# Dylan102938/distributed-llm-inference

Measured on AMD Instinct MI355X. Metric: output tokens/sec (whole node) + p50 token latency, Llama-3-70B PP=8, higher is better.
Workload: dtype bf16; 1 GPU; model=Llama-3-70B, global_batch=512, seq_len=647, parallelism=pp1

## Files before the change

distributed_llm_inference/config.py:

```python
from __future__ import annotations

import dataclasses
import json
import math
import os
from dataclasses import dataclass, field
from typing import Any, Dict, List, Optional, Sequence, Tuple


@dataclass(frozen=True)
class ModelSpec:

    arch: str = "llama"
    vocab_size: int = 128256
    hidden_size: int = 4096
    intermediate_size: int = 14336
    num_layers: int = 32
    num_heads: int = 32
    num_kv_heads: int = 8
    head_dim: int = 128
    rms_norm_eps: float = 1e-5
    rope_theta: float = 500000.0
    rope_scaling: Optional[Tuple[Tuple[str, Any], ...]] = None
    max_position_embeddings: int = 8192
# ... 247 lines not shown
        raise ValueError("num_stages must be >= 1")
    if num_stages > L:
        raise ValueError(f"cannot split {L} layers into {num_stages} stages")
    w = list(weights) if weights is not None else [1.0] * num_stages
    if len(w) != num_stages or min(w) <= 0:
        raise ValueError("weights must be positive, one per stage")
    head_cost = 0.6 * spec.vocab_size * spec.hidden_size / max(1, spec.layer_param_count())
    extra = [0.0] * num_stages
    if num_stages > 1:
        if head_rotation:
            extra = [head_cost / num_stages] * num_stages
        else:
            extra[-1] += head_cost
    total = (L + sum(extra))
    tw = sum(w)
    targets = [total * wi / tw - ei for wi, ei in zip(w, extra)]
    counts = [max(1, int(math.floor(t))) for t in targets]
    while sum(counts) > L:
        i = max((k for k in range(num_stages) if counts[k] > 1),
                key=lambda k: (counts[k] + extra[k]) / w[k])
        counts[i] -= 1
    while sum(counts) < L:
        i = min(range(num_stages), key=lambda k: ((counts[k] + 1 + extra[k]) / w[k], k))
        counts[i] += 1
    out, s = [], 0
    for c in counts:
        out.append((s, s + c))
        s += c
    return out


@dataclass
class CacheConfig:

    block_size: int = 64
    num_blocks: Optional[int] = None
    gpu_memory_utilization: float = 0.90
    window_length: int = 0
    num_sink_tokens: int = 0
    max_chunk: int = 512
    dtype: str = "bf16"
    k_scale: float = 1.0
    v_scale: float = 1.0

    def __post_init__(self):
        if self.dtype not in ("bf16", "fp8"):
            raise ValueError(f"KV cache dtype must be 'bf16' or 'fp8', got {self.dtype!r}")

    @property
    def windowed(self) -> bool:
        return self.window_length > 0

    @property
    def torch_dtype(self):
        import torch
        return torch.float8_e4m3fn if self.dtype == "fp8" else torch.bfloat16

    @property
    def dtype_bytes(self) -> int:
        return 1 if self.dtype == "fp8" else 2


@dataclass
class KernelPolicy:

    gemm4: bool = True
    fp8_gemm4: str = "gate_up"
    gemm4_decode_sched: int = 8
    bf16_partials: bool = True
    defer_splitk: bool = True
    fp8_mx: bool = True
    tile_gemms: bool = True
    library_gemms: Optional[bool] = None
    tile_gemm_max_m: int = 2048
    warm_library_gemms: bool = True
    stream_k_tail: bool = False
    gemv: bool = True
    gemv_norm: bool = True
    int8_transposed: bool = False
    prefill_m32: bool = True
    fp4_mfma: bool = False
    fp4_small_m: int = 0
    fp8_small_m: int = 0

    _FP8_SHAPES = ("qkv", "o", "gate_up", "down")

    def __post_init__(self):
        if self.fp4_small_m != 0 and not 3 <= self.fp4_small_m <= 32:
            raise ValueError(f"fp4_small_m={self.fp4_small_m}: 0 (off) or 3..32")
        if self.fp8_small_m != 0 and not 3 <= self.fp8_small_m <= 32:
            raise ValueError(f"fp8_small_m={self.fp8_small_m}: 0 (off) or 3..32")
        if self.gemm4_decode_sched not in (4, 6, 8, 9):
            raise ValueError(f"gemm4_decode_sched={self.gemm4_decode_sched}: 4, 6, 8 or 9")
        sel = self.fp8_gemm4
        if sel not in ("all", "none") and any(
                x not in self._FP8_SHAPES for x in sel.split("+")):
            raise ValueError(f"fp8_gemm4={sel!r}: 'all', 'none' or a '+' list of "
                             f"{'/'.join(self._FP8_SHAPES)}")

    def fp8_on_gemm4(self, shape: str) -> bool:
        return self.gemm4 and (self.fp8_gemm4 == "all" or shape in self.fp8_gemm4.split("+"))

    def with_overrides(self, spec: str) -> "KernelPolicy":
        if not spec or not spec.strip():
            return self
        kw: Dict[str, Any] = {}
        names = {f.name: f for f in dataclasses.fields(self)}
        for item in spec.split(","):
            if not item.strip():
                continue
            k, _, v = item.partition("=")
            k, v = k.strip(), v.strip()
            if k not in names:
                raise ValueError(f"unknown kernel policy field {k!r} (known: {sorted(names)})")
            if k == "fp8_gemm4":
                kw[k] = v
            elif names[k].type in (int, "int"):
                kw[k] = int(v)
            elif k == "library_gemms" and v.lower() in ("auto", "none", ""):
                kw[k] = None
            elif v.lower() in ("1", "true", "on", "yes"):
                kw[k] = True
            elif v.lower() in ("0", "false", "off", "no"):
                kw[k] = False
            else:
                raise ValueError(f"kernel policy {k}={v!r}: expected 0/1")
        return dataclasses.replace(self, **kw)


@dataclass
class ServeConfig:
    max_batch_size: int = 256
    max_num_batched_tokens: int = 8192
    num_micro_batches: int = 0
    max_seq_len: int = 8192
    use_graphs: bool = True
    head_rotation: bool = True
    graph_batch_sizes: List[int] = field(default_factory=lambda: [1, 2, 4, 8, 16, 32, 64, 96, 128,
                                                                  160, 192, 224, 256])
```

distributed_llm_inference/csrc/bindings.hip:

```cpp
#include <torch/extension.h>
#include <ATen/hip/HIPContext.h>
#include <ATen/hip/impl/HIPGuardImplMasqueradingAsCUDA.h>
#include <ATen/hip/impl/HIPStreamMasqueradingAsCUDA.h>

#include <cstdlib>

#include "kernels/kernels.h"

using at::Tensor;
using c10::optional;

namespace {

#define CHECK_DEV(t) TORCH_CHECK((t).is_cuda(), #t " must be a GPU tensor")
#define CHECK_CONTIG(t) TORCH_CHECK((t).is_contiguous(), #t " must be contiguous")
#define CHECK_BF16(t) TORCH_CHECK((t).scalar_type() == at::kBFloat16, #t " must be bfloat16")
#define CHECK_I32(t) TORCH_CHECK((t).scalar_type() == at::kInt, #t " must be int32")
#define CHECK_I64(t) TORCH_CHECK((t).scalar_type() == at::kLong, #t " must be int64")
#define CHECK_F32(t) TORCH_CHECK((t).scalar_type() == at::kFloat, #t " must be float32")
#define CHECK_IN(t) \
  CHECK_DEV(t);     \
  CHECK_CONTIG(t)

inline dli::bf16* bp(const Tensor& t) { return reinterpret_cast<dli::bf16*>(t.data_ptr()); }
// ... 22 lines not shown
      ro = bp(*residual_out);
    }
  }
  const c10::hip::HIPGuardMasqueradingAsCUDA g(x.device());
  check_rc(dli::launch_rms_norm(bp(out), bp(x), r, ro, bp(w), (float)eps, (int)rows, (int)hidden,
                                cur_stream()), "rms_norm");
}

void splitk_reduce(Tensor out, Tensor parts) {
  CHECK_IN(out); CHECK_IN(parts); CHECK_BF16(out); CHECK_F32(parts);
  TORCH_CHECK(parts.dim() == 3 && out.numel() == parts.size(1) * parts.size(2),
              "splitk_reduce: parts [S, M, N] and out [M, N]");
  const c10::hip::HIPGuardMasqueradingAsCUDA g(parts.device());
  check_rc(dli::launch_splitk_reduce(bp(out), parts.data_ptr<float>(), (int)parts.size(0),
                                     (size_t)out.numel(), cur_stream()), "splitk_reduce");
}

void rms_norm_splitk(Tensor out, Tensor parts, optional<Tensor> residual, Tensor w, double eps,
                     optional<Tensor> residual_out) {
  CHECK_IN(out); CHECK_IN(parts); CHECK_IN(w);
  CHECK_BF16(out); CHECK_BF16(w);
  const bool parts_bf16 = parts.scalar_type() == at::kBFloat16;
  TORCH_CHECK(parts_bf16 || parts.scalar_type() == at::kFloat, "rms_norm_splitk: fp32 or bf16 parts");
  TORCH_CHECK(parts.dim() == 3, "rms_norm_splitk: parts must be [splits, rows, hidden]");
  const int64_t splits = parts.size(0), rows = parts.size(1), hidden = parts.size(2);
  TORCH_CHECK(splits >= 1 && w.numel() == hidden && out.numel() == rows * hidden,
              "rms_norm_splitk: shape mismatch");
  const dli::bf16* r = nullptr;
  dli::bf16* ro = nullptr;
  if (residual.has_value()) {
    CHECK_IN(*residual); CHECK_BF16(*residual);
    TORCH_CHECK(residual->numel() == rows * hidden, "rms_norm_splitk: residual shape mismatch");
    r = bp(*residual);
    ro = bp(*residual);
    if (residual_out.has_value()) {
      CHECK_IN(*residual_out); CHECK_BF16(*residual_out);
      TORCH_CHECK(residual_out->numel() == rows * hidden, "rms_norm_splitk: residual_out shape");
      ro = bp(*residual_out);
    }
  }
  const c10::hip::HIPGuardMasqueradingAsCUDA g(parts.device());
  check_rc(dli::launch_rms_norm(bp(out), nullptr, r, ro, bp(w), (float)eps, (int)rows,
                                (int)hidden, cur_stream(), parts.data_ptr(), (int)splits,
                                parts_bf16),
           "rms_norm_splitk");
}

void layer_norm(Tensor out, Tensor x, optional<Tensor> residual, Tensor w, Tensor b, double eps,
                optional<Tensor> residual_out) {
  CHECK_IN(out); CHECK_IN(x); CHECK_IN(w); CHECK_IN(b);
  CHECK_BF16(out); CHECK_BF16(x); CHECK_BF16(w); CHECK_BF16(b);
  const int64_t hidden = x.size(-1);
  const int64_t rows = x.numel() / hidden;
  TORCH_CHECK(w.numel() == hidden && b.numel() == hidden && out.numel() == x.numel(),
              "layer_norm: shape mismatch");
  const dli::bf16* r = nullptr;
  dli::bf16* ro = nullptr;
  if (residual.has_value()) {
    CHECK_IN(*residual); CHECK_BF16(*residual);
    TORCH_CHECK(residual->numel() == x.numel(), "layer_norm: residual shape mismatch");
    r = bp(*residual);
    ro = bp(*residual);
    if (residual_out.has_value()) {
      CHECK_IN(*residual_out); CHECK_BF16(*residual_out);
      TORCH_CHECK(residual_out->numel() == x.numel(), "layer_norm: residual_out shape mismatch");
      ro = bp(*residual_out);
    }
  }
  const c10::hip::HIPGuardMasqueradingAsCUDA g(x.device());
  check_rc(dli::launch_layer_norm(bp(out), bp(x), r, ro, bp(w), bp(b), (float)eps, (int)rows,
                                  (int)hidden, cur_stream()), "layer_norm");
}

void silu_mul(Tensor out, Tensor x, bool interleaved) {
  CHECK_IN(out); CHECK_IN(x); CHECK_BF16(out); CHECK_BF16(x);
  const int64_t two_i = x.size(-1);
  TORCH_CHECK(two_i % 2 == 0, "silu_mul: last dim must be even");
  const int64_t rows = x.numel() / two_i;
  TORCH_CHECK(out.numel() == rows * (two_i / 2), "silu_mul: out shape mismatch");
  const c10::hip::HIPGuardMasqueradingAsCUDA g(x.device());
  check_rc(dli::launch_silu_mul(bp(out), bp(x), (int)rows, (int)(two_i / 2), interleaved,
                                cur_stream()),
           "silu_mul");
}

void gelu_bias(Tensor out, Tensor x, optional<Tensor> bias) {
  CHECK_IN(out); CHECK_IN(x); CHECK_BF16(out); CHECK_BF16(x);
  const int64_t cols = x.size(-1);
  const int64_t rows = x.numel() / cols;
  TORCH_CHECK(out.numel() == x.numel(), "gelu: out shape mismatch");
  dli::bf16* bb = nullptr;
  if (bias.has_value()) {
    CHECK_IN(*bias); CHECK_BF16(*bias);
    TORCH_CHECK(bias->numel() == cols, "gelu: bias shape mismatch");
    bb = bp(*bias);
  }
  const c10::hip::HIPGuardMasqueradingAsCUDA g(x.device());
  check_rc(dli::launch_gelu_bias(bp(out), bp(x), bb, (int)rows, (int)cols, cur_stream()), "gelu");
}

void add(Tensor out, Tensor a, Tensor b) {
  CHECK_IN(out); CHECK_IN(a); CHECK_IN(b);
  CHECK_BF16(out); CHECK_BF16(a); CHECK_BF16(b);
  TORCH_CHECK(a.numel() == b.numel() && out.numel() == a.numel(), "add: shape mismatch");
  const c10::hip::HIPGuardMasqueradingAsCUDA g(a.device());
  check_rc(dli::launch_add(bp(out), bp(a), bp(b), (size_t)a.numel(), cur_stream()), "add");
}

bool check_cache(const Tensor& k_cache, const Tensor& v_cache, int64_t nkv, int64_t D) {
  CHECK_IN(k_cache); CHECK_IN(v_cache);
  const bool fp8 = k_cache.scalar_type() == at::kFloat8_e4m3fn;
  TORCH_CHECK(fp8 || k_cache.scalar_type() == at::kBFloat16, "KV cache must be bf16 or fp8 e4m3fn");
  TORCH_CHECK(v_cache.scalar_type() == k_cache.scalar_type(), "k/v caches must share a dtype");
  TORCH_CHECK(k_cache.dim() == 4 && v_cache.dim() == 5, "k_cache must be 4-D, v_cache 5-D");
  TORCH_CHECK(k_cache.size(1) == nkv && k_cache.size(3) == D, "k_cache must be [blocks, nkv, bs, D]");
  TORCH_CHECK(v_cache.size(0) == k_cache.size(0) && v_cache.size(1) == nkv &&
                  v_cache.size(2) * 8 == k_cache.size(2) && v_cache.size(3) == D &&
                  v_cache.size(4) == 8,
              "v_cache must be [blocks, nkv, bs/8, D, 8]");
  return fp8;
}

void rope_cache(Tensor qkv, optional<Tensor> positions, optional<Tensor> slot_mapping,
                optional<Tensor> cos_sin, Tensor q_out, optional<Tensor> q_sink_out,
                int64_t window, Tensor k_cache, Tensor v_cache, int64_t nh, int64_t nkv,
                double k_scale, double v_scale) {
  CHECK_DEV(qkv);
  const bool parts_bf16 = qkv.scalar_type() == at::kBFloat16 && qkv.dim() == 3;
  const bool parts = qkv.scalar_type() == at::kFloat || parts_bf16;
  if (parts) {
    TORCH_CHECK(qkv.dim() == 3 && qkv.is_contiguous(), "qkv partials must be contiguous [S, T, N]");
  } else {
    CHECK_BF16(qkv);
    TORCH_CHECK(qkv.dim() == 2 && qkv.stride(1) == 1, "qkv must be [T, *] with unit inner stride");
  }
  const int64_t T = parts ? qkv.size(1) : qkv.size(0);
  CHECK_IN(q_out); CHECK_BF16(q_out);
  TORCH_CHECK(q_out.dim() == 3 && q_out.size(0) == T && q_out.size(1) == nh, "q_out must be [T, nh, D]");
  const int64_t D = q_out.size(2);
  TORCH_CHECK(qkv.size(qkv.dim() - 1) >= (nh + 2 * nkv) * D, "qkv too narrow for nh/nkv/D");
  const bool fp8 = check_cache(k_cache, v_cache, nkv, D);
  TORCH_CHECK(k_scale > 0 && v_scale > 0, "KV scales must be positive");
  dli::RopeCacheParams p{};
  p.kv_fp8 = fp8 ? 1 : 0;
  p.k_inv_scale = (float)(1.0 / k_scale);
  p.v_inv_scale = (float)(1.0 / v_scale);
  if (parts) {
    p.qkv = nullptr;
    p.qkv_parts = qkv.data_ptr();
    p.parts_bf16 = parts_bf16 ? 1 : 0;
    p.splits = (int)qkv.size(0);
    p.qkv_stride = qkv.size(2);
    p.split_stride = (long)(T * qkv.size(2));
  } else {
    p.qkv = bp(qkv);
    p.qkv_stride = qkv.stride(0);
  }
  if (positions.has_value()) {
    CHECK_IN(*positions); CHECK_I32(*positions);
    TORCH_CHECK(positions->numel() == T, "positions must have T entries");
    p.positions = positions->data_ptr<int>();
  }
  if (slot_mapping.has_value()) {
    CHECK_IN(*slot_mapping); CHECK_I64(*slot_mapping);
    TORCH_CHECK(slot_mapping->numel() == T, "slot_mapping must have T entries");
    p.slot_mapping = reinterpret_cast<const long*>(slot_mapping->data_ptr<int64_t>());
// ... 29 lines not shown
                            double k_scale, double v_scale, int64_t& D,
                            bool allow_empty_out = false) {
  CHECK_IN(out); CHECK_IN(q); CHECK_BF16(out); CHECK_BF16(q);
  TORCH_CHECK(q.dim() == 3, "q must be [T, nh, D]");
  TORCH_CHECK(out.sizes() == q.sizes() || (allow_empty_out && out.numel() == 0),
              "out must match q");
  const int64_t nh = q.size(1);
  D = q.size(2);
  const int64_t nkv = k_cache.size(1);
  TORCH_CHECK(nkv > 0 && nh % nkv == 0, "nh must be a multiple of nkv");
  const bool fp8 = check_cache(k_cache, v_cache, nkv, D);
  TORCH_CHECK(k_scale > 0 && v_scale > 0, "KV scales must be positive");
  CHECK_IN(block_tables); CHECK_I32(block_tables); CHECK_IN(seq_lens); CHECK_I32(seq_lens);
  TORCH_CHECK(block_tables.dim() == 2 && block_tables.size(0) == seq_lens.size(0),
              "block_tables must be [B, max_blocks]");
  dli::AttnParams p{};
  p.q = bp(q);
  if (ring > 0) {
    TORCH_CHECK(q_sink.has_value() || n_sink == 0, "window mode with sinks needs q_sink");
    TORCH_CHECK(window > n_sink && sink_pad >= n_sink && sink_pad % 32 == 0 && ring % 32 == 0,
                "invalid window configuration");
  }
  if (q_sink.has_value()) {
    CHECK_IN(*q_sink); CHECK_BF16(*q_sink);
    TORCH_CHECK(q_sink->sizes() == q.sizes(), "q_sink must match q");
    p.q_sink = bp(*q_sink);
  }
  p.k_cache = k_cache.data_ptr();
  p.v_cache = v_cache.data_ptr();
  p.kv_fp8 = fp8 ? 1 : 0;
  p.k_scale = (float)k_scale;
  p.v_scale = (float)v_scale;
  p.out = out.numel() ? bp(out) : nullptr;
  p.block_tables = block_tables.data_ptr<int>();
  p.bt_stride = (int)block_tables.size(1);
  p.seq_lens = seq_lens.data_ptr<int>();
  p.scale_log2 = (float)(scale * 1.4426950408889634);
  p.nh = (int)nh;
  p.nkv = (int)nkv;
  p.bs = (int)k_cache.size(2);
  p.n_sink = (int)n_sink;
  p.sink_pad = (int)sink_pad;
  p.ring = (int)ring;
  p.window = (int)window;
  p.num_splits = 1;
  TORCH_CHECK(p.bs % 32 == 0, "cache block size must be a multiple of 32");
  return p;
}

void attn_decode(Tensor out, Tensor q, optional<Tensor> q_sink, Tensor k_cache, Tensor v_cache,
                 Tensor block_tables, Tensor seq_lens, double scale, int64_t n_sink,
                 int64_t sink_pad, int64_t ring, int64_t window, int64_t num_splits,
                 optional<Tensor> part_o, optional<Tensor> part_ml, double k_scale,
                 double v_scale, optional<Tensor> out_q, optional<Tensor> out_mx) {
  int64_t D = 0;
  auto p = attn_common(out, q, q_sink, k_cache, v_cache, block_tables, seq_lens, scale, n_sink,
                       sink_pad, ring, window, k_scale, v_scale, D, out_q.has_value());
  const int64_t B = q.size(0);
  TORCH_CHECK(seq_lens.numel() == B, "decode: one token per sequence (seq_lens must have T entries)");
  TORCH_CHECK(num_splits >= 1, "num_splits >= 1");
  p.num_splits = (int)num_splits;
  TORCH_CHECK(out_q.has_value() == out_mx.has_value(), "attn_decode: out_q and out_mx go together");
  if (out_q.has_value()) {
    CHECK_IN(*out_q); CHECK_IN(*out_mx);
    TORCH_CHECK(D == 128 && num_splits == 1, "attn_decode: MX output needs head_dim 128, one split");
    TORCH_CHECK(out_q->element_size() == 1 && out_q->numel() == B * p.nh * D,
                "attn_decode: out_q = fp8 [T, nh * D]");
    TORCH_CHECK(out_mx->element_size() == 1 && out_mx->numel() == p.nh * ((B + 63) / 64) * 64,
                "attn_decode: out_mx = e8m0 [nh][ceil(T / 64) * 64]");
    p.out_q = static_cast<uint8_t*>(out_q->data_ptr());
    p.out_mx = static_cast<uint8_t*>(out_mx->data_ptr());
  }
  if (num_splits > 1) {
    TORCH_CHECK(part_o.has_value() && part_ml.has_value(), "split-K needs workspaces");
    CHECK_IN(*part_o); CHECK_IN(*part_ml); CHECK_F32(*part_o); CHECK_F32(*part_ml);
    TORCH_CHECK(part_o->numel() >= num_splits * B * p.nh * D, "part_o workspace too small");
    TORCH_CHECK(part_ml->numel() >= num_splits * B * p.nh * 2, "part_ml workspace too small");
    p.part_o = part_o->data_ptr<float>();
    p.part_ml = part_ml->data_ptr<float>();
  }
  const c10::hip::HIPGuardMasqueradingAsCUDA g(q.device());
  check_rc(dli::launch_attn_decode(p, (int)B, (int)D, cur_stream()), "attn_decode");
}

void attn_prefill(Tensor out, Tensor q, optional<Tensor> q_sink, Tensor k_cache, Tensor v_cache,
                  Tensor block_tables, Tensor seq_lens, Tensor q_start, int64_t max_q,
                  double scale, int64_t n_sink, int64_t sink_pad, int64_t ring, int64_t window,
                  double k_scale, double v_scale, optional<Tensor> tile_map, int64_t qb,
                  optional<Tensor> mask, bool m32) {
  int64_t D = 0;
  auto p = attn_common(out, q, q_sink, k_cache, v_cache, block_tables, seq_lens, scale, n_sink,
                       sink_pad, ring, window, k_scale, v_scale, D);
  CHECK_IN(q_start); CHECK_I32(q_start);
  const int64_t B = seq_lens.numel();
  TORCH_CHECK(q_start.numel() == B + 1, "q_start must have B+1 entries");
  p.q_start = q_start.data_ptr<int>();
  if (tile_map.has_value()) {
    CHECK_IN(*tile_map); CHECK_I32(*tile_map);
    TORCH_CHECK(tile_map->dim() == 2 && tile_map->size(1) == 2, "tile_map must be [n_tiles, 2]");
    p.tile_map = tile_map->data_ptr<int>();
    p.n_tiles = (int)tile_map->size(0);
  }
  TORCH_CHECK(qb == 1 || qb == 2, "attn_prefill: qb (query blocks per wave) must be 1 or 2");
  p.prefill_qb = (int)qb;
  p.prefill_m32 = m32 ? 1 : 0;
  if (mask.has_value()) {
    CHECK_IN(*mask); CHECK_F32(*mask);
    TORCH_CHECK(mask->dim() == 4 && mask->size(0) == B &&
                    (mask->size(1) == 1 || mask->size(1) == q.size(1)),
                "attn_prefill: mask must be [B, 1 | nh, T, keys]");
    TORCH_CHECK(ring == 0 && !tile_map.has_value(),
                "attn_prefill: a custom mask needs a full cache and the dense grid");
    p.mask = mask->data_ptr<float>();
    p.mask_heads = (int)mask->size(1);
    p.mask_q = (int)mask->size(2);
    p.mask_k = (int)mask->size(3);
  }
  const c10::hip::HIPGuardMasqueradingAsCUDA g(q.device());
  check_rc(dli::launch_attn_prefill(p, (int)B, (int)max_q, (int)D, cur_stream()), "attn_prefill");
}

void sample(Tensor out_tokens, optional<Tensor> out_logprobs, Tensor logits,
            optional<Tensor> temperature, optional<Tensor> top_k, optional<Tensor> top_p,
            optional<Tensor> seeds, optional<Tensor> step, optional<Tensor> ctr) {
  CHECK_DEV(logits);
  TORCH_CHECK(logits.dim() == 2 && logits.stride(1) == 1, "logits must be [B, V] row-major");
  TORCH_CHECK(logits.scalar_type() == at::kBFloat16 || logits.scalar_type() == at::kFloat,
              "logits must be bf16 or f32");
  const int64_t B = logits.size(0);
  CHECK_IN(out_tokens); CHECK_I32(out_tokens);
  TORCH_CHECK(out_tokens.numel() == B, "out_tokens must have B entries");
  dli::SampleParams p{};
  p.logits = logits.data_ptr();
  p.logits_is_f32 = logits.scalar_type() == at::kFloat;
  p.row_stride = logits.stride(0);
  p.V = (int)logits.size(1);
  auto opt_f = [&](optional<Tensor>& t, const char* n) -> const float* {
    if (!t.has_value()) return nullptr;
    CHECK_IN(*t); CHECK_F32(*t);
    TORCH_CHECK(t->numel() == B, n, " must have B entries");
    return t->data_ptr<float>();
  };
  p.temperature = opt_f(temperature, "temperature");
  p.top_p = opt_f(top_p, "top_p");
  if (top_k.has_value()) {
    CHECK_IN(*top_k); CHECK_I32(*top_k);
    TORCH_CHECK(top_k->numel() == B, "top_k must have B entries");
    p.top_k = top_k->data_ptr<int>();
  }
  if (seeds.has_value()) {
    CHECK_IN(*seeds); CHECK_I64(*seeds);
    TORCH_CHECK(seeds->numel() == B, "seeds must have B entries");
    p.seeds = reinterpret_cast<const unsigned long long*>(seeds->data_ptr<int64_t>());
  }
  if (step.has_value()) {
    CHECK_IN(*step); CHECK_I64(*step);
    p.step = reinterpret_cast<const long*>(step->data_ptr<int64_t>());
  }
  if (ctr.has_value()) {
    CHECK_IN(*ctr); CHECK_I64(*ctr);
    TORCH_CHECK(ctr->numel() == B, "ctr must have B entries");
    p.ctr = reinterpret_cast<const long*>(ctr->data_ptr<int64_t>());
  }
  p.out_tokens = out_tokens.data_ptr<int>();
  if (out_logprobs.has_value()) {
    CHECK_IN(*out_logprobs); CHECK_F32(*out_logprobs);
// ... 606 lines not shown
  }
  TORCH_CHECK(M >= 1 && M <= 2 && (fp4 || w.size(1) == K) && q_out.size(0) == M &&
                  q_out.size(1) == nh && N == (nh + 2 * nkv) * D,
              "skinny_gemm_qkv_rope: x [M <= 2, K], w [(nh + 2 nkv) D, K], q_out [M, nh, D]");
  const bool fp8 = check_cache(k_cache, v_cache, nkv, D);
  TORCH_CHECK(k_scale > 0 && v_scale > 0, "KV scales must be positive");
  dli::GemvRope rp{};
  rp.kv_fp8 = fp8 ? 1 : 0;
  rp.k_inv_scale = (float)(1.0 / k_scale);
  rp.v_inv_scale = (float)(1.0 / v_scale);
  if (positions.has_value()) {
    CHECK_IN(*positions); CHECK_I32(*positions);
    TORCH_CHECK(positions->numel() == M, "positions must have M entries");
    rp.positions = positions->data_ptr<int>();
  }
  if (slot_mapping.has_value()) {
    CHECK_IN(*slot_mapping); CHECK_I64(*slot_mapping);
    TORCH_CHECK(slot_mapping->numel() == M, "slot_mapping must have M entries");
    rp.slot_mapping = reinterpret_cast<const long*>(slot_mapping->data_ptr<int64_t>());
  }
  if (cos_sin.has_value()) {
    CHECK_IN(*cos_sin); CHECK_F32(*cos_sin);
    TORCH_CHECK(cos_sin->dim() == 2 && cos_sin->size(1) == D && positions.has_value(),
                "cos_sin must be [max_pos, D] (with positions)");
    rp.cos_sin = cos_sin->data_ptr<float>();
    rp.max_pos = (int)cos_sin->size(0);
  }
  rp.q_out = bp(q_out);
  rp.k_cache = k_cache.data_ptr();
  rp.v_cache = v_cache.data_ptr();
  rp.nh = (int)nh;
  rp.nkv = (int)nkv;
  rp.D = (int)D;
  rp.bs = (int)k_cache.size(2);
  const GemvNormArgs na = gemv_norm_args(x, norm_w, res_in, res_out, eps, "skinny_gemm_qkv_rope");
  const dli::GemvNorm* nm = na.on ? &na.nm : nullptr;
  const dli::bf16* b = nullptr;
  if (bias.has_value()) {
    CHECK_IN(*bias); CHECK_BF16(*bias);
    TORCH_CHECK(bias->numel() == N, "skinny_gemm_qkv_rope: bias must have N entries");
    b = bp(*bias);
  }
  const c10::hip::HIPGuardMasqueradingAsCUDA g(x.device());
  int rc;
  if (fp4) {
    rc = dli::launch_skinny_gemm_fp4(nullptr, bp(x), w.data_ptr<uint8_t>(),
                                     block_scale->data_ptr<uint8_t>(), b, (int)M, (int)N, (int)K,
                                     cur_stream(), false, nm, &rp);
  } else if (w.scalar_type() == at::kBFloat16) {
    rc = dli::launch_skinny_gemm(nullptr, bp(x), bp(w), b, (int)M, (int)N, (int)K, cur_stream(),
                                 false, nm, &rp);
  } else {
    TORCH_CHECK(wscale.has_value() && w.element_size() == 1, "8-bit weights need wscale");
    CHECK_IN(*wscale); CHECK_F32(*wscale);
    TORCH_CHECK(wscale->numel() == N, "wscale must have N entries");
    if (w.scalar_type() == at::kChar)
      rc = dli::launch_skinny_gemm_int8(nullptr, bp(x), w.data_ptr<int8_t>(),
                                        wscale->data_ptr<float>(), b, (int)M, (int)N, (int)K,
                                        cur_stream(), false, nm, &rp);
    else
      rc = dli::launch_skinny_gemm_fp8(nullptr, x.data_ptr(), nullptr,
                                       static_cast<const uint8_t*>(w.data_ptr()),
                                       wscale->data_ptr<float>(), b, (int)M, (int)N, (int)K,
                                       cur_stream(), false, nm, &rp);
  }
  check_rc(rc, "skinny_gemm_qkv_rope");
}


}

void register_rccl(pybind11::module_& m);
void register_streams(pybind11::module_& m);

PYBIND11_MODULE(TORCH_EXTENSION_NAME, m) {
  m.doc() = "CDNA4 (gfx950) kernels of distributed_llm_inference";
  m.def("rms_norm", &rms_norm, "RMSNorm (+fused residual add)", py::arg("out"), py::arg("x"),
        py::arg("residual"), py::arg("w"), py::arg("eps"), py::arg("residual_out") = py::none());
  m.def("layer_norm", &layer_norm, "LayerNorm (+fused residual add)", py::arg("out"),
        py::arg("x"), py::arg("residual"), py::arg("w"), py::arg("b"), py::arg("eps"),
        py::arg("residual_out") = py::none());
  m.def("silu_mul", &silu_mul, "SwiGLU: out = silu(x[:, :I]) * x[:, I:] (or tile-interleaved)",
        py::arg("out"), py::arg("x"), py::arg("interleaved") = false);
  m.def("gelu_bias", &gelu_bias, "gelu_tanh(x + bias)");
  m.def("add", &add, "out = a + b");
  m.def("rope_cache", &rope_cache, "fused RoPE + paged KV cache write");
  m.def("attn_decode", &attn_decode, "paged GQA decode attention (split-K)", py::arg("out"),
        py::arg("q"), py::arg("q_sink"), py::arg("k_cache"), py::arg("v_cache"),
        py::arg("block_tables"), py::arg("seq_lens"), py::arg("scale"), py::arg("n_sink"),
        py::arg("sink_pad"), py::arg("ring"), py::arg("window"), py::arg("num_splits"),
        py::arg("part_o"), py::arg("part_ml"), py::arg("k_scale"), py::arg("v_scale"),
        py::arg("out_q") = py::none(), py::arg("out_mx") = py::none());
  m.def("attn_prefill", &attn_prefill, "paged causal prefill attention (varlen)", py::arg("out"),
        py::arg("q"), py::arg("q_sink"), py::arg("k_cache"), py::arg("v_cache"),
        py::arg("block_tables"), py::arg("seq_lens"), py::arg("q_start"), py::arg("max_q"),
        py::arg("scale"), py::arg("n_sink"), py::arg("sink_pad"), py::arg("ring"),
        py::arg("window"), py::arg("k_scale"), py::arg("v_scale"), py::arg("tile_map"),
        py::arg("qb"), py::arg("mask") = py::none(), py::arg("m32") = true);
  m.def("sample", &sample, "greedy / temperature / top-k / top-p sampling", py::arg("out_tokens"),
        py::arg("out_logprobs"), py::arg("logits"), py::arg("temperature"), py::arg("top_k"),
        py::arg("top_p"), py::arg("seeds"), py::arg("step"), py::arg("ctr") = py::none());
  m.def("digest", &digest, "hop-integrity payload digest partials", py::arg("part"), py::arg("t"));
  m.def("quant_rowwise", &quant_rowwise, "row-wise fp8 e4m3 quantisation (+fused RMSNorm)",
        py::arg("q_out"), py::arg("scale"), py::arg("x"), py::arg("residual"), py::arg("norm_w"),
        py::arg("eps"), py::arg("residual_out") = py::none());
  m.def("quant_rowwise_int8", &quant_rowwise_int8, "LLM.int8 row-wise int8 quantisation (outlier columns zeroed)",
        py::arg("q_out"), py::arg("scale"), py::arg("x"), py::arg("outlier") = py::none());
  m.def("llm_int8_outliers", &llm_int8_outliers,
        "LLM.int8 outlier columns: (flags, x_out, w_out, cnt) for the bf16 outlier product",
        py::arg("x"), py::arg("wq"), py::arg("ws"), py::arg("threshold"), py::arg("max_out"),
        py::arg("wq_t") = py::none(), py::arg("dynamic") = false);
  m.def("silu_mul_quant", &silu_mul_quant, "SwiGLU fused with row-wise fp8 quantisation");
  m.def("gemm_tile", &gemm_tile, "C = A . B^T, 256x256 LDS-DMA 8-phase MFMA tile GEMM",
        py::arg("out"), py::arg("a"), py::arg("b"), py::arg("splits") = 1,
        py::arg("epilogue") = 0, py::arg("workspace") = py::none(),
        py::arg("a_scale") = py::none(), py::arg("b_scale") = py::none(),
        py::arg("x_out") = py::none(), py::arg("w_out") = py::none(),
        py::arg("a_mx") = py::none(), py::arg("out_mx") = py::none(),
        py::arg("ol_cnt") = py::none());
  m.def("rms_norm_splitk", &rms_norm_splitk, "residual add + RMSNorm over un-reduced split-K partials",
        py::arg("out"), py::arg("parts"), py::arg("residual"), py::arg("w"), py::arg("eps"),
        py::arg("residual_out") = py::none());
  m.def("splitk_reduce", &splitk_reduce, "bf16 out = sum of fp32 split-K partials [S, M, N]");
  m.def("gemm_tile_sk_workspace_floats", []() { return dli::gemm_tile_sk_workspace_floats(); },
        "fp32 workspace elements gemm_tile(splits=0) needs on the current device");
  m.def("skinny_gemm_qkv_rope", &skinny_gemm_qkv_rope,
        "1-2 row fused QKV GEMV with RoPE + paged KV write in its epilogue (+ fused input RMSNorm)",
        py::arg("q_out"), py::arg("x"), py::arg("w"), py::arg("wscale"), py::arg("bias"),
        py::arg("positions"), py::arg("slot_mapping"), py::arg("cos_sin"), py::arg("k_cache"),
        py::arg("v_cache"), py::arg("nh"), py::arg("nkv"), py::arg("k_scale") = 1.0,
        py::arg("v_scale") = 1.0, py::arg("norm_w") = py::none(), py::arg("res_in") = py::none(),
        py::arg("res_out") = py::none(), py::arg("eps") = 1e-5,
        py::arg("block_scale") = py::none());
  m.def("skinny_gemm_fp4", &skinny_gemm_fp4,
        "y = x . dequant(W4)^T (+ bias), MXFP4 weights, bf16 rows, M <= 2 (weight-streaming GEMV)",
        py::arg("out"), py::arg("x"), py::arg("w"), py::arg("block_scale"),
        py::arg("bias") = py::none(), py::arg("swiglu") = false, py::arg("norm_w") = py::none(),
        py::arg("res_in") = py::none(), py::arg("res_out") = py::none(), py::arg("eps") = 1e-5);
  m.def("small_gemm_fp4", &small_gemm_fp4,
        "y = x . dequant(W4)^T (+ bias), MXFP4 weights, 3-32 bf16 rows (weight-streaming MFMA GEMM)",
        py::arg("out"), py::arg("x"), py::arg("w"), py::arg("block_scale"),
        py::arg("bias") = py::none(), py::arg("swiglu") = false);
  m.def("small_gemm_fp8", &small_gemm_fp8,
        "y = (x . W8^T) * w_scale (+ bias), fp8 weights, 3-32 bf16 rows (weight-streaming MFMA GEMM)",
        py::arg("out"), py::arg("x"), py::arg("w"), py::arg("w_scale"),
        py::arg("bias") = py::none(), py::arg("swiglu") = false);
  m.def("dequant_mxfp4", &dequant_mxfp4, "bf16 [N, K] = MXFP4 nibbles [N, K / 2] * 2^(e8m0 - 127)",
        py::arg("out"), py::arg("w"), py::arg("block_scale"));
  m.def("quant_mx", &quant_mx, "MX fp8 quantiser: bf16 [M, K] -> e4m3 bytes + e8m0 per (row, 128)",
        py::arg("q"), py::arg("sc"), py::arg("x"));
  m.def("gemm_fp4", &gemm_fp4,
        "C = A . W^T, MX fp8 activations x MXFP4 weights on the mixed-format block-scaled MFMA",
        py::arg("out"), py::arg("a_q"), py::arg("a_mx"), py::arg("w"), py::arg("block_scale"),
        py::arg("splits") = 1, py::arg("epilogue") = 0, py::arg("workspace") = py::none());
  m.def("gemm_fp4_max_ktiles", []() { return dli::gemm_fp4_max_ktiles(); },
        "k-tiles (of 128) one split of gemm_fp4 may own");
  m.def("gemm4", &gemm4, "C = A . B^T, one-wave-per-SIMD 256x256 MFMA tile GEMM (gemm4.hip)",
        py::arg("out"), py::arg("a"), py::arg("b"), py::arg("splits") = 1,
        py::arg("epilogue") = 0, py::arg("grid") = 0, py::arg("a_scale") = py::none(),
        py::arg("b_scale") = py::none(), py::arg("variant") = -1, py::arg("a_mx") = py::none(),
        py::arg("out_mx") = py::none());
  m.def("skinny_gemm_int8", &skinny_gemm_int8,
        "y = (x . W8^T) * scale (+ bias), int8 weights, bf16 rows, M <= 2 (weight-streaming GEMV)",
        py::arg("out"), py::arg("x"), py::arg("w"), py::arg("wscale"), py::arg("bias") = py::none(),
        py::arg("swiglu") = false, py::arg("norm_w") = py::none(), py::arg("res_in") = py::none(),
        py::arg("res_out") = py::none(), py::arg("eps") = 1e-5);
  m.def("skinny_gemm_fp8", &skinny_gemm_fp8,
        "y = (x . W8^T) * scale (+ bias), fp8 e4m3 weights, M <= 2 (weight-streaming GEMV)",
        py::arg("out"), py::arg("x"), py::arg("xscale"), py::arg("w"), py::arg("wscale"),
        py::arg("bias") = py::none(), py::arg("swiglu") = false, py::arg("norm_w") = py::none(),
        py::arg("res_in") = py::none(), py::arg("res_out") = py::none(), py::arg("eps") = 1e-5);
  m.def("skinny_gemm", &skinny_gemm, "y = x . W^T (+ bias) for M <= 4 (weight-streaming GEMV)",
        py::arg("out"), py::arg("x"), py::arg("w"), py::arg("bias") = py::none(),
        py::arg("swiglu") = false, py::arg("norm_w") = py::none(), py::arg("res_in") = py::none(),
        py::arg("res_out") = py::none(), py::arg("eps") = 1e-5);
// ... 4 lines not shown
```

distributed_llm_inference/csrc/kernels/activation.hip:

```cpp
#include "kernels.h"

namespace dli {

template <bool INTERLEAVED>
__global__ void __launch_bounds__(256) silu_mul_kernel(bf16* __restrict__ out,
                                                       const bf16* __restrict__ x, int rows,
                                                       int inter) {
  const int nvec = inter >> 3;
  const size_t total = (size_t)rows * nvec;
  for (size_t i = blockIdx.x * (size_t)blockDim.x + threadIdx.x; i < total;
       i += (size_t)gridDim.x * blockDim.x) {
    const size_t r = i / nvec, c = i % nvec;
    const bf16* row = x + r * 2 * inter;
    bf16x8 g, u;
    if (INTERLEAVED) {
      const int o = (int)c * 8;
      const int gc = (o >> 7) * 256 + ((o & 127) >> 5) * 64 + ((o & 31) >> 4) * 32 + (o & 15);
      g = *reinterpret_cast<const bf16x8*>(row + gc);
      u = *reinterpret_cast<const bf16x8*>(row + gc + 16);
    } else {
      g = reinterpret_cast<const bf16x8*>(row)[c];
      u = reinterpret_cast<const bf16x8*>(row + inter)[c];
    }
    bf16x8 o;
#pragma unroll
    for (int j = 0; j < 8; ++j) o[j] = (bf16)(silu((float)g[j]) * (float)u[j]);
    reinterpret_cast<bf16x8*>(out + r * inter)[c] = o;
  }
}

__global__ void __launch_bounds__(256) gelu_bias_kernel(bf16* __restrict__ out,
                                                        const bf16* __restrict__ x,
                                                        const bf16* __restrict__ bias, int rows,
                                                        int cols) {
  const int nvec = cols >> 3;
  const size_t total = (size_t)rows * nvec;
  for (size_t i = blockIdx.x * (size_t)blockDim.x + threadIdx.x; i < total;
       i += (size_t)gridDim.x * blockDim.x) {
    const size_t c = i % nvec;
    const bf16x8 a = reinterpret_cast<const bf16x8*>(x)[i];
    bf16x8 o;
    if (bias) {
      const bf16x8 b = reinterpret_cast<const bf16x8*>(bias)[c];
#pragma unroll
      for (int j = 0; j < 8; ++j) o[j] = (bf16)gelu_tanh((float)a[j] + (float)b[j]);
    } else {
#pragma unroll
      for (int j = 0; j < 8; ++j) o[j] = (bf16)gelu_tanh((float)a[j]);
    }
    reinterpret_cast<bf16x8*>(out)[i] = o;
  }
}

__global__ void __launch_bounds__(256) add_kernel(bf16* __restrict__ out, const bf16* __restrict__ a,
                                                  const bf16* __restrict__ b, size_t nvec) {
  for (size_t i = blockIdx.x * (size_t)blockDim.x + threadIdx.x; i < nvec;
       i += (size_t)gridDim.x * blockDim.x) {
    const bf16x8 x = reinterpret_cast<const bf16x8*>(a)[i];
    const bf16x8 y = reinterpret_cast<const bf16x8*>(b)[i];
    bf16x8 o;
#pragma unroll
    for (int j = 0; j < 8; ++j) o[j] = (bf16)((float)x[j] + (float)y[j]);
    reinterpret_cast<bf16x8*>(out)[i] = o;
  }
}

static inline int ew_grid(size_t work) {
  size_t g = (work + 255) / 256;
  if (g > 2048) g = 2048;
  if (g < 1) g = 1;
  return (int)g;
}

int launch_silu_mul(bf16* out, const bf16* x, int rows, int inter, bool interleaved,
                    hipStream_t stream) {
  if (inter % 8 != 0 || (interleaved && inter % 128 != 0)) return -1;
  if (rows == 0) return 0;
  if (interleaved)
    silu_mul_kernel<true><<<ew_grid((size_t)rows * inter / 8), 256, 0, stream>>>(out, x, rows, inter);
  else
    silu_mul_kernel<false><<<ew_grid((size_t)rows * inter / 8), 256, 0, stream>>>(out, x, rows, inter);
  return 0;
}

int launch_gelu_bias(bf16* out, const bf16* x, const bf16* bias, int rows, int cols,
                     hipStream_t stream) {
  if (cols % 8 != 0) return -1;
  if (rows == 0) return 0;
  gelu_bias_kernel<<<ew_grid((size_t)rows * cols / 8), 256, 0, stream>>>(out, x, bias, rows, cols);
  return 0;
}

int launch_add(bf16* out, const bf16* a, const bf16* b, size_t n, hipStream_t stream) {
  if (n % 8 != 0) return -1;
  if (n == 0) return 0;
  add_kernel<<<ew_grid(n / 8), 256, 0, stream>>>(out, a, b, n / 8);
  return 0;
}

}
```

distributed_llm_inference/csrc/kernels/attention.hip:

```cpp
#include "kernels.h"
#include "attn_core.h"

#include <type_traits>

namespace dli {

template <int D, bool WIN, bool FP8, bool GRP, bool ONE = false>
__global__ void __launch_bounds__(256, (ONE ? 4 : 1))
attn_decode_kernel(AttnParams p, int items, int gs) {
  constexpr int LROW = D + 4;
  __shared__ __attribute__((aligned(16))) float lds[GRP ? 4 * 16 * (LROW + 2) : 1];
  const int wave = threadIdx.x >> 6;
  const int item_raw = blockIdx.x * 4 + wave;
  const bool live = item_raw < items;
  if (!GRP && !live) return;
  const int item = __builtin_amdgcn_readfirstlane(live ? item_raw : items - 1);
  WaveState<D> st;
  const DecodeItem di = attn_decode_item<D, WIN, FP8, false, ONE>(p, item, live, st);
  const int splits = p.num_splits, split = di.split, G = di.G, hgroups = di.hgroups;
  const int g0 = di.g0, kvh = di.kvh, b = di.b;
  const int lane = threadIdx.x & 63, col = lane & 15, h4 = lane >> 4;
  const bool col_valid = di.col_valid;
  const float vsc = di.vsc;
  float lsum = st.l;
  lsum += __shfl_xor(lsum, 16, 64);
  lsum += __shfl_xor(lsum, 32, 64);
  const size_t B = (size_t)items / ((size_t)splits * hgroups * p.nkv);
  if constexpr (!GRP) {
    if (!col_valid) return;
    const int head = kvh * G + g0 + col;
    if (splits == 1) {
      const float inv = lsum > 0.f ? vsc / lsum : 0.f;
      if constexpr (D == 128) {
        if (p.out_q != nullptr) {
          f32x4 vals[D / 16];
          int dd[D / 16];
          float a = 0.f;
#pragma unroll
          for (int u = 0; u < D / 16; ++u) {
            f32x4 o;
            o_unit<D, FP8>(st, u, h4, dd[u], o);
#pragma unroll
            for (int r = 0; r < 4; ++r) {
              vals[u][r] = (float)(bf16)(o[r] * inv);
              a = fmaxf(a, fabsf(vals[u][r]));
            }
          }
          a = fmaxf(a, __shfl_xor(a, 16, 64));
          a = fmaxf(a, __shfl_xor(a, 32, 64));
          const int k = mx_exponent(a);
          const float si = mx_inv_scale(k);
          uint8_t* qrow = p.out_q + ((size_t)b * p.nh + head) * D;
#pragma unroll
          for (int u = 0; u < D / 16; ++u) {
            const f32x4 v = vals[u] * si;
            *reinterpret_cast<unsigned*>(qrow + dd[u]) = pack4_fp8(v[0], v[1], v[2], v[3]);
          }
          if (h4 == 0) {
            const int nb = ((int)B + 63) / 64;
            p.out_mx[mx_off(head, b, nb)] = (uint8_t)(k + 127);
            if (b == (int)B - 1)
              for (int r = (int)B; r < nb * 64; ++r) p.out_mx[mx_off(head, r, nb)] = 127;
          }
          return;
        }
      }
      bf16* orow = p.out + ((size_t)b * p.nh + head) * D;
#pragma unroll
      for (int u = 0; u < D / 16; ++u) {
        int d;
        f32x4 o;
        o_unit<D, FP8>(st, u, h4, d, o);
        bf16x4 v;
#pragma unroll
        for (int r = 0; r < 4; ++r) v[r] = (bf16)(o[r] * inv);
        *reinterpret_cast<bf16x4*>(orow + d) = v;
      }
    } else {
      const size_t r0 = ((size_t)split * B + b) * p.nh + head;
      float* prow = p.part_o + r0 * D;
#pragma unroll
      for (int u = 0; u < D / 16; ++u) {
        int d;
        f32x4 o;
        o_unit<D, FP8>(st, u, h4, d, o);
        *reinterpret_cast<f32x4*>(prow + d) = o * vsc;
      }
      if (h4 == 0) {
        p.part_ml[r0 * 2] = st.m;
        p.part_ml[r0 * 2 + 1] = lsum;
      }
    }
  } else {
    float* lo = lds + (wave * 16 + col) * LROW;
    float* lml = lds + 4 * 16 * LROW;
#pragma unroll
    for (int u = 0; u < D / 16; ++u) {
      int d;
      f32x4 o;
      o_unit<D, FP8>(st, u, h4, d, o);
      *reinterpret_cast<f32x4*>(lo + d) = o;
// ... 286 lines not shown
    for (int qb = 0; qb < QB; ++qb) {
      if constexpr (MASK) {
        const int k0 = u0 + 8 * h4;
        float madd[8];
        unsigned vis = 0;
#pragma unroll
        for (int j = 0; j < 8; ++j) {
          const float mv = k0 + j < mlen ? mrow[k0 + j] : -INFINITY;
          const bool ok = mv > -1e4f;
          madd[j] = ok ? mv * minv : 0.f;
          vis |= (ok ? 1u : 0u) << j;
        }
        attn_core<D>(st[qb], qf[qb], f, sl2, [&](int j) { return ((vis >> j) & 1u) != 0; },
                     [&](int j) { return madd[j]; });
        continue;
      }
      if constexpr (!WIN) {
        attn_compute_causal<D>(st[qb], qf[qb], f, sl2, pq[qb] - (u0 + 8 * h4));
        continue;
      }
      unsigned vm = 0;
#pragma unroll
      for (int j = 0; j < 8; ++j) {
        const int u = u0 + 8 * h4 + j;
        bool ok;
        if (!WIN) {
          ok = u <= pq[qb];
        } else if (sink_step) {
          ok = u < nS && u <= pq[qb];
        } else {
          ok = (u - p.sink_pad) < seg_len;
          if (ok) {
            const int a = ring_abs(u, L, p);
            ok = a >= p.n_sink && a <= pq[qb] && (pq[qb] - a) < (p.window - p.n_sink);
          }
        }
        vm |= (ok ? 1u : 0u) << j;
      }
      if constexpr (WIN) {
        if (sink_step) {
          attn_compute<D>(st[qb], qsf[qb], f, sl2, vm);
          continue;
        }
      }
      attn_compute<D>(st[qb], qf[qb], f, sl2, vm);
    }
    if constexpr (DMA) {
      asm volatile("s_waitcnt vmcnt(0)" ::: "memory");
    } else {
      if (sidx + 1 < nsteps) swrite(buf ^ 1);
    }
    __syncthreads();
  }
#pragma unroll
  for (int qb = 0; qb < QB; ++qb) {
    float lsum = st[qb].l;
    lsum += __shfl_xor(lsum, 16, 64);
    lsum += __shfl_xor(lsum, 32, 64);
    if (col_valid[qb]) {
      const float inv = lsum > 0.f ? vsc / lsum : 0.f;
      bf16* orow = p.out + ((size_t)(qs0 + tok[qb]) * p.nh + qh) * D;
#pragma unroll
      for (int e = 0; e < D / 16; ++e) {
        bf16x4 v;
#pragma unroll
        for (int r = 0; r < 4; ++r) v[r] = (bf16)(st[qb].o[e][r] * inv);
        *reinterpret_cast<bf16x4*>(orow + 16 * e + 4 * h4) = v;
      }
    }
  }
}

static int attn_cus() {
  static int cus = [] {
    int dev = 0, n = 0;
    if (hipGetDevice(&dev) != hipSuccess ||
        hipDeviceGetAttribute(&n, hipDeviceAttributeMultiprocessorCount, dev) != hipSuccess || n <= 0)
      return 256;
    return n;
  }();
  return cus;
}

template <int D, bool WIN, bool FP8>
static void decode_grid(const AttnParams& p, int items, int gs, hipStream_t stream) {
  const int grid = (items + 3) / 4;
  if (p.num_splits > 1) {
    attn_decode_kernel<D, WIN, FP8, true><<<grid, 256, 0, stream>>>(p, items, gs);
    return;
  }
  if constexpr (!WIN) {
#ifndef ATTN_DECODE_TWO_STEP
    const long s1 = 16L * attn_cus(), s2 = 8L * attn_cus();
    const long r1 = (items + s1 - 1) / s1, r2 = (items + s2 - 1) / s2;
    if (items >= s1 && (double)items / (r1 * s1) >= (double)items / (r2 * s2)) {
      attn_decode_kernel<D, WIN, FP8, false, true><<<grid, 256, 0, stream>>>(p, items, 1);
      return;
    }
#endif
  }
  attn_decode_kernel<D, WIN, FP8, false><<<grid, 256, 0, stream>>>(p, items, 1);
}

template <int D>
static int launch_decode_d(const AttnParams& p, int B, hipStream_t stream) {
  const int G = p.nh / p.nkv;
  const int hgroups = (G + 15) / 16;
  const long items = (long)B * p.nkv * hgroups * p.num_splits;
  if (items > (1L << 30)) return -3;
  const int gs = p.num_splits % 4 == 0 ? 4 : p.num_splits % 2 == 0 ? 2 : 1;
  if (p.ring > 0) {
    if (p.kv_fp8) decode_grid<D, true, true>(p, (int)items, gs, stream);
    else decode_grid<D, true, false>(p, (int)items, gs, stream);
  } else {
    if (p.kv_fp8) decode_grid<D, false, true>(p, (int)items, gs, stream);
    else decode_grid<D, false, false>(p, (int)items, gs, stream);
  }
  if (p.num_splits > gs) {
    AttnParams pc = p;
    pc.num_splits = p.num_splits / gs;
    attn_combine_kernel<D><<<B * p.nh, 256, 0, stream>>>(pc, B);
  }
  return 0;
}

int launch_attn_decode(const AttnParams& p, int B, int D, hipStream_t stream) {
  if (B == 0) return 0;
  if (p.bs % 32 != 0 || (p.ring > 0 && (p.sink_pad % 32 != 0 || p.ring % 32 != 0))) return -2;
  switch (D) {
    case 32: return launch_decode_d<32>(p, B, stream);
    case 64: return launch_decode_d<64>(p, B, stream);
    case 128: return launch_decode_d<128>(p, B, stream);
    default: return -1;
  }
}

template <int D, bool WIN, bool FP8>
static void prefill_grid(const AttnParams& p, dim3 grid, int hpw, hipStream_t stream) {
  if constexpr (!WIN) {
    if (p.mask) {
      attn_prefill_kernel<D, false, FP8, 1, true><<<grid, 256, 0, stream>>>(p, hpw);
      return;
    }
  }
  if (p.prefill_qb == 2)
    attn_prefill_kernel<D, WIN, FP8, 2><<<grid, 256, 0, stream>>>(p, hpw);
  else
    attn_prefill_kernel<D, WIN, FP8, 1><<<grid, 256, 0, stream>>>(p, hpw);
}

template <int D>
static int launch_prefill_d(const AttnParams& p, int B, int max_q, hipStream_t stream) {
  const int G = p.nh / p.nkv;
  const int hpw = (G % 4 == 0) ? 4 : (G % 2 == 0 ? 2 : 1);
  const int tpw = 4 / hpw;
  const int tt = 16 * tpw * (p.mask ? 1 : p.prefill_qb);
  dim3 grid((max_q + tt - 1) / tt, p.nkv * (G / hpw), B);
  if (p.tile_map) {
    const long total = (long)p.n_tiles * p.nkv * (G / hpw);
    grid = dim3((unsigned)((total + 7) / 8 * 8), 1, 1);
  }
  if (grid.x == 0) return 0;
  if (p.ring > 0) {
    if (p.kv_fp8) prefill_grid<D, true, true>(p, grid, hpw, stream);
    else prefill_grid<D, true, false>(p, grid, hpw, stream);
  } else {
    if (p.kv_fp8) prefill_grid<D, false, true>(p, grid, hpw, stream);
    else prefill_grid<D, false, false>(p, grid, hpw, stream);
  }
  return 0;
}

int launch_attn_prefill(const AttnParams& p, int B, int max_q, int D, hipStream_t stream) {
  if (B == 0 || max_q == 0) return 0;
  if (p.prefill_qb != 1 && p.prefill_qb != 2) return -3;
  if (p.bs % 32 != 0 || (p.ring > 0 && (p.sink_pad % 32 != 0 || p.ring % 32 != 0))) return -2;
  if (p.mask && (p.ring > 0 || p.tile_map || p.mask_heads < 1 || p.mask_q < 1 || p.mask_k < 1))
    return -4;
  if (attn_prefill32_eligible(p, D)) return launch_attn_prefill32(p, B, max_q, stream);
  switch (D) {
    case 32: return launch_prefill_d<32>(p, B, max_q, stream);
    case 64: return launch_prefill_d<64>(p, B, max_q, stream);
    case 128: return launch_prefill_d<128>(p, B, max_q, stream);
    default: return -1;
  }
}

}
```

distributed_llm_inference/csrc/kernels/attn_core.h:

```cpp
#pragma once
#include "kernels.h"

namespace dli {

typedef int i32x4 __attribute__((ext_vector_type(4)));

__device__ __forceinline__ int bt_entry(const int* bt, int i) {
  const int* a = bt + __builtin_amdgcn_readfirstlane(i);
  int v;
  asm volatile("s_load_dword %0, %1, 0x0\n\ts_waitcnt lgkmcnt(0)" : "=s"(v) : "s"(a));
  return v;
}

__device__ __forceinline__ bf16x8 zero8() {
  i32x4 z = {0, 0, 0, 0};
  return __builtin_bit_cast(bf16x8, z);
}

__device__ __forceinline__ f32x4 mfma16(const bf16x8& a, const bf16x8& b, const f32x4& c) {
  return __builtin_amdgcn_mfma_f32_16x16x32_bf16(a, b, c, 0, 0, 0);
}

__device__ __forceinline__ int ring_abs(int u, int L, const AttnParams& p) {
  const int o = u - p.sink_pad;
  const int newest = (L - 1 - p.n_sink) % p.ring;
  int back = newest - o;
  if (back < 0) back += p.ring;
  return (L - 1) - back;
}

template <int D>
struct WaveState {
  f32x4 o[D / 16];
  float m, l;
  __device__ __forceinline__ void init() {
#pragma unroll
    for (int e = 0; e < D / 16; ++e) o[e] = f32x4{0.f, 0.f, 0.f, 0.f};
    m = -1e30f;
    l = 0.f;
  }
};

template <int D>
struct KVFrag {
  bf16x8 k[2][D / 32];
  bf16x8 v[D / 16];
};

template <int D, bool FP8>
struct DPerm {
  static constexpr bool on = FP8 && D % 64 == 0;
};

template <int D, bool FP8>
__device__ __forceinline__ int q_dofs(int c, int h4) {
  return DPerm<D, FP8>::on ? 64 * (c >> 1) + 16 * h4 + 8 * (c & 1) : 32 * c + 8 * h4;
}

template <bool NT>
__device__ __forceinline__ bf16x8 kv_ld16(const bf16* p) {
  if constexpr (NT) {
    typedef int i32x4_t __attribute__((ext_vector_type(4)));
    return __builtin_bit_cast(bf16x8, __builtin_nontemporal_load(reinterpret_cast<const i32x4_t*>(p)));
  } else {
    return *reinterpret_cast<const bf16x8*>(p);
  }
}

template <int D, bool FP8, bool NT = false>
__device__ __forceinline__ void attn_load(KVFrag<D>& f, const void* __restrict__ kc,
                                          const void* __restrict__ vc, size_t hb, int offk,
                                          int nvalid = 32) {
  const int lane = threadIdx.x & 63;
  const int col = lane & 15, h4 = lane >> 4;
  const int krow0 = offk + 8 * (col >> 2) + (col & 3);
  if constexpr (DPerm<D, FP8>::on) {
    const uint8_t* k8 = static_cast<const uint8_t*>(kc);
    const uint8_t* v8 = static_cast<const uint8_t*>(vc);
#pragma unroll
    for (int t = 0; t < 2; ++t)
#pragma unroll
      for (int c2 = 0; c2 < D / 64; ++c2) {
        const uint4 r = *reinterpret_cast<const uint4*>(k8 + hb + (size_t)(krow0 + 4 * t) * D + 64 * c2 + 16 * h4);
        f.k[t][2 * c2] = fp8x8_to_bf16x8(make_uint2(r.x, r.y));
// ... 91 lines not shown
__device__ __forceinline__ void attn_core(WaveState<D>& st, const bf16x8 (&qf)[D / 32],
                                          const KVFrag<D>& f, float scale_log2, Visible visible,
                                          Bias bias = Bias()) {
  f32x4 s[2];
#pragma unroll
  for (int t = 0; t < 2; ++t) {
    s[t] = f32x4{0.f, 0.f, 0.f, 0.f};
#pragma unroll
    for (int c = 0; c < D / 32; ++c) s[t] = mfma16(f.k[t][c], qf[c], s[t]);
  }
  float x[8];
  float mx = -INFINITY;
#pragma unroll
  for (int j = 0; j < 8; ++j) {
    x[j] = visible(j) ? s[j >> 2][j & 3] + bias(j) : -INFINITY;
    mx = fmaxf(mx, x[j]);
  }
  mx = fmaxf(mx, __shfl_xor(mx, 16, 64));
  mx = fmaxf(mx, __shfl_xor(mx, 32, 64));
  const float m_new = fmaxf(st.m, mx * scale_log2);
  const float alpha = __builtin_amdgcn_exp2f(st.m - m_new);
  bf16x8 pb;
  float ps = 0.f;
#pragma unroll
  for (int j = 0; j < 8; ++j) {
    const float pj = __builtin_amdgcn_exp2f(fmaf(x[j], scale_log2, -m_new));
    ps += pj;
    pb[j] = (bf16)pj;
  }
  st.l = st.l * alpha + ps;
  st.m = m_new;
#pragma unroll
  for (int e = 0; e < D / 16; ++e) {
    st.o[e] *= alpha;
    st.o[e] = mfma16(f.v[e], pb, st.o[e]);
  }
}

template <int D>
__device__ __forceinline__ void attn_compute(WaveState<D>& st, const bf16x8 (&qf)[D / 32],
                                             const KVFrag<D>& f, float scale_log2,
                                             unsigned valid_mask) {
  attn_core<D>(st, qf, f, scale_log2, [&](int j) { return ((valid_mask >> j) & 1u) != 0; });
}

template <int D>
__device__ __forceinline__ void attn_compute_causal(WaveState<D>& st, const bf16x8 (&qf)[D / 32],
                                                    const KVFrag<D>& f, float scale_log2, int lim) {
  attn_core<D>(st, qf, f, scale_log2, [&](int j) { return j <= lim; });
}

template <int D, bool FP8>
__device__ __forceinline__ void attn_step(WaveState<D>& st, const bf16x8 (&qf)[D / 32],
                                          const void* kc, const void* vc, size_t hb, int offk,
                                          float scale_log2, unsigned valid_mask) {
  KVFrag<D> f;
  attn_load<D, FP8>(f, kc, vc, hb, offk);
  attn_compute<D>(st, qf, f, scale_log2, valid_mask);
}

template <int D, bool WIN>
__device__ __forceinline__ unsigned step_mask(int u0, int h4, int seg_base, int seg_len, int L,
                                              const AttnParams& p) {
  unsigned vm = 0;
#pragma unroll
  for (int j = 0; j < 8; ++j) {
    const int u = u0 + 8 * h4 + j;
    bool ok = (u - seg_base) < seg_len;
    if (WIN && ok) {
      const int a = ring_abs(u, L, p);
      ok = a >= p.n_sink && (L - 1 - a) < (p.window - p.n_sink);
    }
    vm |= (ok ? 1u : 0u) << j;
  }
  return vm;
}

struct DecodeItem {
  int split, b, kvh, g0, G, hgroups;
  bool col_valid;
  float vsc;
};

template <int D, bool WIN, bool FP8, bool NT, bool ONE_STEP = false>
__device__ __forceinline__ DecodeItem attn_decode_item(const AttnParams& p, int item, bool live,
                                                       WaveState<D>& st) {
  const int splits = p.num_splits;
  const int split = item % splits;
  int rest = item / splits;
  const int G = p.nh / p.nkv;
  const int hgroups = (G + 15) >> 4;
  const int g0 = (rest % hgroups) * 16;
  rest /= hgroups;
  const int kvh = rest % p.nkv;
  const int b = rest / p.nkv;
  const int lane = threadIdx.x & 63;
  const int col = lane & 15, h4 = lane >> 4;
  const bool col_valid = (g0 + col) < G;
  const int qh = kvh * G + g0 + (col_valid ? col : 0);
  const int L = live ? p.seq_lens[b] : 0;
  const int* bt = p.block_tables + (size_t)b * p.bt_stride;
  const size_t head_stride = (size_t)p.bs * D;

  const float sl2 = FP8 ? p.scale_log2 * p.k_scale : p.scale_log2;
  const float vsc = FP8 ? p.v_scale : 1.f;
  st.init();
  if (L > 0) {
    bf16x8 qf[D / 32];
    const bf16* qrow = p.q + ((size_t)b * p.nh + qh) * D;
#pragma unroll
    for (int c = 0; c < D / 32; ++c)
      qf[c] = col_valid ? *reinterpret_cast<const bf16x8*>(qrow + q_dofs<D, FP8>(c, h4)) : zero8();
    int seg_base, seg_len;
    if (WIN) {
      seg_base = p.sink_pad;
      seg_len = L > p.n_sink ? min(p.ring, L - p.n_sink) : 0;
    } else {
      seg_base = 0;
      seg_len = L;
    }
    const int nsteps = (seg_len + 31) >> 5;
    const int per_split = (nsteps + splits - 1) / splits;
    const int s_lo = split * per_split;
    const int s_hi = min(nsteps, s_lo + per_split);
    if (s_lo < s_hi) {
      auto load = [&](KVFrag<D>& f, int sidx) {
        const int u0 = seg_base + sidx * 32;
        const int page = bt_entry(bt, u0 / p.bs);
        const size_t hb = ((size_t)page * p.nkv + kvh) * head_stride;
        attn_load<D, FP8, NT>(f, p.k_cache, p.v_cache, hb, u0 % p.bs,
                              WIN ? 32 : seg_len - sidx * 32);
      };
      if constexpr (DPerm<D, FP8>::on) {
        auto rload = [&](KVRaw<D>& r, int sidx) {
          const int u0 = seg_base + sidx * 32;
          const int page = bt_entry(bt, u0 / p.bs);
          const size_t hb = ((size_t)page * p.nkv + kvh) * head_stride;
          attn_load_raw<D>(r, p.k_cache, p.v_cache, hb, u0 % p.bs);
        };
        auto step = [&](const KVRaw<D>& r, int sidx) {
          KVFrag<D> f;
          attn_widen<D>(f, r);
          attn_compute<D>(st, qf, f, sl2,
                          step_mask<D, WIN>(seg_base + sidx * 32, h4, seg_base, seg_len, L, p));
        };
        if constexpr (ONE_STEP) {
          for (int sidx = s_lo; sidx < s_hi; ++sidx) {
            KVRaw<D> r;
            rload(r, sidx);
            step(r, sidx);
          }
        } else {
        KVRaw<D> r0, r1, r2;
        rload(r0, s_lo);
        rload(r1, min(s_lo + 1, s_hi - 1));
        for (int sidx = s_lo; sidx < s_hi; sidx += 3) {
          rload(r2, min(sidx + 2, s_hi - 1));
          __builtin_amdgcn_sched_barrier(0);
          step(r0, sidx);
          rload(r0, min(sidx + 3, s_hi - 1));
          __builtin_amdgcn_sched_barrier(0);
          if (sidx + 1 < s_hi) step(r1, sidx + 1);
          rload(r1, min(sidx + 4, s_hi - 1));
          __builtin_amdgcn_sched_barrier(0);
          if (sidx + 2 < s_hi) step(r2, sidx + 2);
        }
        }
      } else {
      if constexpr (ONE_STEP) {
        for (int sidx = s_lo; sidx < s_hi; ++sidx) {
          KVFrag<D> f;
          load(f, sidx);
          attn_compute<D>(st, qf, f, sl2,
                          step_mask<D, WIN>(seg_base + sidx * 32, h4, seg_base, seg_len, L, p));
        }
      } else {
      KVFrag<D> fa, fb;
      load(fa, s_lo);
      for (int sidx = s_lo; sidx < s_hi; sidx += 2) {
        load(fb, min(sidx + 1, s_hi - 1));
        __builtin_amdgcn_sched_barrier(0);
        attn_compute<D>(st, qf, fa, sl2,
                        step_mask<D, WIN>(seg_base + sidx * 32, h4, seg_base, seg_len, L, p));
        load(fa, min(sidx + 2, s_hi - 1));
        __builtin_amdgcn_sched_barrier(0);
        if (sidx + 1 < s_hi)
          attn_compute<D>(st, qf, fb, sl2,
                          step_mask<D, WIN>(seg_base + (sidx + 1) * 32, h4, seg_base, seg_len, L, p));
      }
      }
      }
    }
    if (WIN && split == 0 && p.n_sink > 0) {
      bf16x8 qs[D / 32];
      const bf16* qsrow = p.q_sink + ((size_t)b * p.nh + qh) * D;
#pragma unroll
      for (int c = 0; c < D / 32; ++c)
        qs[c] = col_valid ? *reinterpret_cast<const bf16x8*>(qsrow + q_dofs<D, FP8>(c, h4)) : zero8();
      const int nS = min(p.n_sink, L);
      for (int u0 = 0; u0 < nS; u0 += 32) {
        const int page = bt_entry(bt, u0 / p.bs);
        const size_t hb = ((size_t)page * p.nkv + kvh) * head_stride;
        unsigned vm = 0;
#pragma unroll
        for (int j = 0; j < 8; ++j) vm |= ((u0 + 8 * h4 + j) < nS ? 1u : 0u) << j;
        attn_step<D, FP8>(st, qs, p.k_cache, p.v_cache, hb, u0 % p.bs, sl2, vm);
      }
    }
  }
  DecodeItem di;
  di.split = split;
  di.b = b;
  di.kvh = kvh;
  di.g0 = g0;
  di.G = G;
  di.hgroups = hgroups;
  di.col_valid = col_valid;
  di.vsc = vsc;
  return di;
}

}
```

distributed_llm_inference/csrc/kernels/common.h:

```cpp
#pragma once
#include <hip/hip_runtime.h>
#include <stdint.h>

namespace dli {

typedef __bf16 bf16;
typedef __bf16 bf16x8 __attribute__((ext_vector_type(8)));
typedef __bf16 bf16x4 __attribute__((ext_vector_type(4)));
typedef __bf16 bf16x2 __attribute__((ext_vector_type(2)));
typedef float f32x4 __attribute__((ext_vector_type(4)));
typedef float f32x16 __attribute__((ext_vector_type(16)));
typedef float f32x2 __attribute__((ext_vector_type(2)));

constexpr int kWave = 64;
constexpr float kLog2e = 1.4426950408889634f;

__device__ __forceinline__ int lane_id() { return threadIdx.x & 63; }
__device__ __forceinline__ int wave_id() { return threadIdx.x >> 6; }

template <typename T>
__device__ __forceinline__ T wave_reduce_sum(T v) {
#pragma unroll
  for (int o = 32; o > 0; o >>= 1) v += __shfl_xor(v, o, 64);
  return v;
// ... 98 lines not shown
  }
}

template <int NS>
__device__ __forceinline__ bf16 sum_parts1(const bf16* p, size_t stride) {
  float s = (float)p[0];
#pragma unroll
  for (int k = 1; k < NS; ++k) s += (float)p[k * stride];
  return (bf16)s;
}

__device__ __forceinline__ int row_vec_idx(int i, int nvec) {
  const int idx = (int)threadIdx.x + i * (int)blockDim.x;
  return idx < nvec ? idx : nvec - 1;
}
__device__ __forceinline__ bool row_valid(int i, int nvec) {
  return (int)threadIdx.x + i * (int)blockDim.x < nvec;
}

template <int VPT, int NS, bool PB>
__device__ __forceinline__ void load_row_vecs(bf16x8 (&a)[VPT], const bf16* x, const void* parts,
                                              size_t row_off, size_t stride, int nvec) {
  if constexpr (NS == 0) {
    const bf16x8* xr = reinterpret_cast<const bf16x8*>(x + row_off);
#pragma unroll
    for (int i = 0; i < VPT; ++i) a[i] = xr[row_vec_idx(i, nvec)];
  } else {
    constexpr int CH0 = PB ? 16 / NS : 8 / NS;
    constexpr int CH = CH0 < 1 ? 1 : (CH0 > VPT ? VPT : CH0);
#pragma unroll
    for (int c = 0; c < VPT; c += CH) {
      if constexpr (PB) {
        const bf16* pp = static_cast<const bf16*>(parts) + row_off;
        bf16x8 r[CH][NS];
#pragma unroll
        for (int i = 0; i < CH; ++i)
#pragma unroll
          for (int k = 0; k < NS; ++k)
            if (c + i < VPT)
              r[i][k] = *reinterpret_cast<const bf16x8*>(
                  pp + k * stride + (size_t)row_vec_idx(c + i, nvec) * 8);
#pragma unroll
        for (int i = 0; i < CH; ++i)
          if (c + i < VPT)
#pragma unroll
            for (int j = 0; j < 8; ++j) {
              float sm = (float)r[i][0][j];
#pragma unroll
              for (int k = 1; k < NS; ++k) sm += (float)r[i][k][j];
              a[c + i][j] = (bf16)sm;
            }
      } else {
        const float* pp = static_cast<const float*>(parts) + row_off;
        f32x4 r0[CH][NS], r1[CH][NS];
#pragma unroll
        for (int i = 0; i < CH; ++i)
#pragma unroll
          for (int k = 0; k < NS; ++k)
            if (c + i < VPT) {
              const float* q = pp + k * stride + (size_t)row_vec_idx(c + i, nvec) * 8;
              r0[i][k] = *reinterpret_cast<const f32x4*>(q);
              r1[i][k] = *reinterpret_cast<const f32x4*>(q + 4);
            }
#pragma unroll
        for (int i = 0; i < CH; ++i)
          if (c + i < VPT) {
            f32x4 s0 = r0[i][0], s1 = r1[i][0];
#pragma unroll
            for (int k = 1; k < NS; ++k) {
              s0 += r0[i][k];
              s1 += r1[i][k];
            }
#pragma unroll
            for (int j = 0; j < 4; ++j) {
              a[c + i][j] = (bf16)s0[j];
              a[c + i][j + 4] = (bf16)s1[j];
            }
          }
      }
    }
  }
}

#define SPLITS_SWITCH(splits, MACRO) \
  switch (splits) {                      \
    case 0: MACRO(0); break;             \
    case 1: MACRO(1); break;             \
    case 2: MACRO(2); break;             \
    case 3: MACRO(3); break;             \
    case 4: MACRO(4); break;             \
    case 5: MACRO(5); break;             \
    case 6: MACRO(6); break;             \
    case 7: MACRO(7); break;             \
    case 8: MACRO(8); break;             \
    default: return -2;                  \
  }

__device__ __forceinline__ float block_reduce_sum(float v, float* scratch) {
  v = wave_reduce_sum(v);
  const int nw = blockDim.x >> 6;
  if (lane_id() == 0) scratch[wave_id()] = v;
  __syncthreads();
  float r = 0.f;
  for (int i = 0; i < nw; ++i) r += scratch[i];
  __syncthreads();
  return r;
}

__device__ __forceinline__ float block_reduce_max(float v, float* scratch) {
  v = wave_reduce_max(v);
  const int nw = blockDim.x >> 6;
  if (lane_id() == 0) scratch[wave_id()] = v;
  __syncthreads();
  float r = -INFINITY;
  for (int i = 0; i < nw; ++i) r = fmaxf(r, scratch[i]);
  __syncthreads();
  return r;
}

__device__ __forceinline__ unsigned pack4_fp8(float a, float b, float c, float d) {
  int r = 0;
  r = __builtin_amdgcn_cvt_pk_fp8_f32(a, b, r, false);
  r = __builtin_amdgcn_cvt_pk_fp8_f32(c, d, r, true);
  return (unsigned)r;
}

__device__ __forceinline__ size_t mx_off(int kt, int r, int nb) {
  return ((size_t)kt * nb + (r >> 6)) * 64 + (r & 15) * 4 + ((r & 63) >> 4);
}

__device__ __forceinline__ int mx_exponent(float amax) {
  int k = 0;
  if (amax > 0.f) {
    const unsigned bits = __float_as_uint(amax / 448.f);
    k = (int)((bits >> 23) & 0xff) - 127 + ((bits & 0x7fffff) ? 1 : 0);
    k = min(max(k, -126), 126);
  }
  return k;
}
__device__ __forceinline__ float mx_inv_scale(int k) {
  return __uint_as_float((unsigned)(127 - k) << 23);
}

__device__ __forceinline__ bf16x8 fp8x8_to_bf16x8(uint2 v) {
  typedef __bf16 bf16x2_t __attribute__((ext_vector_type(2)));
  const bf16x2_t a = __builtin_amdgcn_cvt_scalef32_pk_bf16_fp8(v.x, 1.0f, false);
  const bf16x2_t b = __builtin_amdgcn_cvt_scalef32_pk_bf16_fp8(v.x, 1.0f, true);
  const bf16x2_t c = __builtin_amdgcn_cvt_scalef32_pk_bf16_fp8(v.y, 1.0f, false);
  const bf16x2_t d = __builtin_amdgcn_cvt_scalef32_pk_bf16_fp8(v.y, 1.0f, true);
  bf16x8 o;
  o[0] = a[0]; o[1] = a[1]; o[2] = b[0]; o[3] = b[1];
  o[4] = c[0]; o[5] = c[1]; o[6] = d[0]; o[7] = d[1];
  return o;
}

__device__ __forceinline__ uint8_t f32_to_fp8(float x) {
  return (uint8_t)(__builtin_amdgcn_cvt_pk_fp8_f32(x, 0.f, 0, false) & 0xff);
}

__device__ __forceinline__ float silu(float x) { return x / (1.f + __expf(-x)); }

__device__ __forceinline__ float gelu_tanh(float x) {
  const float k0 = 0.7978845608028654f, k1 = 0.044715f;
  return 0.5f * x * (1.f + tanhf(k0 * (x + k1 * x * x * x)));
}

}

#define CHECK_HIP(expr)                                                         \
  do {                                                                              \
    hipError_t _e = (expr);                                                         \
    if (_e != hipSuccess) {                                                         \
      fprintf(stderr, "HIP error %s at %s:%d\n", hipGetErrorString(_e), __FILE__, \
              __LINE__);                                                            \
      abort();                                                                      \
    }                                                                               \
  } while (0)
```

distributed_llm_inference/csrc/kernels/gemm4.hip:

```cpp
#include "kernels.h"

#include <type_traits>
#include <utility>

namespace dli {

namespace {

#ifndef GEMM4_A_AUX
#define GEMM4_A_AUX 0
#endif
#ifndef GEMM4_B_AUX
#define GEMM4_B_AUX 0
#endif

constexpr int kG4Threads = 256;
constexpr int kG4Stage = 65536;

enum G4Epi { kG4Bf16 = 0, kG4F32 = 1, kG4SwiGLU = 2, kG4SwiGLUMx = 3, kG4Bf16Part = 4 };

constexpr int kG4MxKt = 64;
constexpr int kG4MxLds = kG4MxKt * 256;
static_assert(kG4MxLds == 4 * 256 * 16, "the MX slab load: 4 x 16 B per lane of 256 lanes");
constexpr int kG4RedLds = 2 * 256 * 4;

struct G4Mx {
  const uint8_t* a_sc;
  uint8_t* out_sc;
  int nb;
};

typedef __attribute__((address_space(3))) void g4_lds_t;

template <bool V>
struct G4B { static constexpr bool value = V; };

template <typename F, int... I>
__device__ __forceinline__ void g4_static_for(std::integer_sequence<int, I...>, F&& f) {
  (f(std::integral_constant<int, I>{}), ...);
}

template <int V> struct G4Sched;
template <> struct G4Sched<4> {
  static constexpr int q0 = 0, qs = 2, b1 = 35, d0 = 36, ds = 4, b2 = 104, vm = 16, p0 = 105, ps = 1;
};
template <> struct G4Sched<6> {
  static constexpr int q0 = 0, qs = 2, b1 = 35, d0 = 36, ds = 6, b2 = 104, vm = 12, p0 = 105, ps = 1;
};
template <> struct G4Sched<8> : G4Sched<4> { static constexpr bool nt = true; };
template <> struct G4Sched<9> : G4Sched<6> { static constexpr bool nt = true; };
template <typename S, typename = void> struct G4BFirst { static constexpr bool value = false; };
template <typename S> struct G4BFirst<S, std::void_t<decltype(S::bfirst)>> {
  static constexpr bool value = S::bfirst;
};
template <int V, typename = void> struct G4Nt { static constexpr bool value = false; };
template <int V> struct G4Nt<V, std::void_t<decltype(G4Sched<V>::nt)>> {
  static constexpr bool value = G4Sched<V>::nt;
};
constexpr int kG4Default = 4, kG4DecodeDefault = 8;

__device__ __forceinline__ float g4_silu(float x) { return x / (1.f + __expf(-x)); }

__device__ __forceinline__ void g4_mfma(f32x4& acc, const bf16x8& w, const bf16x8& x) {
  asm volatile("v_mfma_f32_16x16x32_bf16 %0, %1, %2, %0" : "+a"(acc) : "v"(w), "v"(x) : "memory");
}

typedef int g4_i32x4 __attribute__((ext_vector_type(4)));
typedef int g4_i32x8 __attribute__((ext_vector_type(8)));
typedef float g4_f32x16 __attribute__((ext_vector_type(16)));

__device__ __forceinline__ void g4_mfma8(f32x4& acc, const g4_i32x4& w0, const g4_i32x4& w1,
                                         const g4_i32x4& x0, const g4_i32x4& x1, int sc) {
  const g4_i32x8 w = __builtin_shufflevector(w0, w1, 0, 1, 2, 3, 4, 5, 6, 7);
  const g4_i32x8 x = __builtin_shufflevector(x0, x1, 0, 1, 2, 3, 4, 5, 6, 7);
  asm volatile("v_mfma_scale_f32_16x16x128_f8f6f4 %0, %1, %2, %0, %3, %3 op_sel_hi:[0,0,0]"
               : "+a"(acc) : "v"(w), "v"(x), "v"(sc) : "memory");
}

template <int SEL>
__device__ __forceinline__ void g4_mfma8mx(f32x4& acc, const g4_i32x4& w0, const g4_i32x4& w1,
                                           const g4_i32x4& x0, const g4_i32x4& x1, int sc, int sx) {
  const g4_i32x8 w = __builtin_shufflevector(w0, w1, 0, 1, 2, 3, 4, 5, 6, 7);
  const g4_i32x8 x = __builtin_shufflevector(x0, x1, 0, 1, 2, 3, 4, 5, 6, 7);
  if constexpr (SEL == 0)
    asm volatile("v_mfma_scale_f32_16x16x128_f8f6f4 %0, %1, %2, %0, %3, %4 op_sel_hi:[0,0,0]"
                 : "+a"(acc) : "v"(w), "v"(x), "v"(sc), "v"(sx) : "memory");
  else if constexpr (SEL == 1)
    asm volatile("v_mfma_scale_f32_16x16x128_f8f6f4 %0, %1, %2, %0, %3, %4 op_sel:[0,1,0] op_sel_hi:[0,0,0]"
                 : "+a"(acc) : "v"(w), "v"(x), "v"(sc), "v"(sx) : "memory");
  else if constexpr (SEL == 2)
    asm volatile("v_mfma_scale_f32_16x16x128_f8f6f4 %0, %1, %2, %0, %3, %4 op_sel_hi:[0,1,0]"
                 : "+a"(acc) : "v"(w), "v"(x), "v"(sc), "v"(sx) : "memory");
  else
    asm volatile("v_mfma_scale_f32_16x16x128_f8f6f4 %0, %1, %2, %0, %3, %4 op_sel:[0,1,0] op_sel_hi:[0,1,0]"
                 : "+a"(acc) : "v"(w), "v"(x), "v"(sc), "v"(sx) : "memory");
}

template <int V> struct G4S8;
template <> struct G4S8<0> {
  static constexpr int la = 7, b1 = 5, d0 = 6, ds = 2, b2 = 37, vm = 16, p0 = 38;
};
template <> struct G4S8<1> {
  static constexpr int la = 5, b1 = 8, d0 = 9, ds = 2, b2 = 40, vm = 16, p0 = 41;
};
template <> struct G4S8<2> {
  static constexpr int la = 7, b1 = 5, d0 = 6, ds = 3, b2 = 40, vm = 12, p0 = 41;
};
constexpr int kG8Default = 0, kG8Variants = 3;
template <typename S> struct G4S8Reads {
  static constexpr int n = 16 + 2 * S::la;
  static constexpr int len = 64 - S::p0;
  static constexpr int lo(int g) { return g < S::p0 ? 0 : ((g - S::p0) * n + len - 1) / len; }
  static constexpr int pos(int r) { return S::p0 + r * len / n; }
  static constexpr bool ok() {
    for (int i = 1; i < S::la; ++i)
      if (pos(18 + 2 * (i - 1)) < 8 * i + 9) return false;
    return S::b1 >= 2 * (8 - S::la) && S::d0 > S::b1 && S::d0 + (S::vm - 1) * S::ds <= S::b2 &&
           (S::vm == 16 || S::d0 + S::vm * S::ds > S::b2) && S::p0 > S::b2 &&
           S::d0 + 15 * S::ds <= 63 && 2 * (S::la - 1) <= 15;
  }
};
static_assert(G4S8Reads<G4S8<0>>::ok() && G4S8Reads<G4S8<1>>::ok() && G4S8Reads<G4S8<2>>::ok(),
              "fp8 k-loop schedule violates a hazard / count constraint");

typedef unsigned g4_u32x2 __attribute__((ext_vector_type(2)));

__device__ __forceinline__ void g4_read_mx(g4_u32x2& dst, int addr) {
  asm volatile("ds_read2_b32 %0, %1 offset1:16" : "=v"(dst) : "v"(addr) : "memory");
}

template <int OFF>
__device__ __forceinline__ void g4_read8(g4_i32x4& dst, int addr) {
  asm volatile("ds_read_b128 %0, %1 offset:%2" : "=v"(dst) : "v"(addr), "i"(OFF) : "memory");
}

template <int OFF>
__device__ __forceinline__ void g4_read(bf16x8& dst, int addr) {
  asm volatile("ds_read_b128 %0, %1 offset:%2" : "=v"(dst) : "v"(addr), "i"(OFF) : "memory");
}

__device__ __forceinline__ void g4_sync_lds() { asm volatile("s_waitcnt lgkmcnt(0)" ::: "memory"); }
__device__ __forceinline__ void g4_barrier() { asm volatile("s_barrier" ::: "memory"); }

#ifdef GEMM_PROBE
// ... 307 lines not shown
          if (DMA) g4_barrier();
#ifdef GEMM_PROBE
          G4P_FENCE(pr.t4); G4P_FENCE(pr.t5); G4P_FENCE(pr.t0);
          pr.ew += pr.t5 - pr.t4;
          pr.t4 = pr.t5 = 0;
          G4P_TIME(pr.t1);
#endif
        }
        if constexpr (DMA && g >= S::d0 && g < S::d0 + 16 * S::ds && (g - S::d0) % S::ds == 0)
          dma(t + 2, G4BFirst<S>::value ? (((g - S::d0) / S::ds) + 8) & 15 : (g - S::d0) / S::ds);
        if constexpr (NEXT && g == S::b2) {
#ifdef GEMM_PROBE
          unsigned long long t2, t3;
          G4P_TIME(t2);
#endif
          if (DMA) g4_vmcnt<S::vm>(); else g4_vmcnt<0>();
          g4_barrier();
#ifdef GEMM_PROBE
          G4P_TIME(t3);
          g4_sync_lds();
          G4P_FENCE(t2); G4P_FENCE(t3); G4P_FENCE(pr.t1);
          pr.b2 += t3 - t2;
          pr.b1 += pr.t1 - pr.t0;
          pr.t0 = pr.t1 = 0;
#endif
        }
        if constexpr (NEXT && g >= S::p0 && g < S::p0 + 16 * S::ps && (g - S::p0) % S::ps == 0)
          rd(P, (g - S::p0) / S::ps, 0, s ^ 1);
      });
#ifdef GEMM_PROBE
      if (NEXT) G4P_TIME(pr.t4);
#endif
      if (NEXT) g4_sync_lds();
#ifdef GEMM_PROBE
      if (NEXT) G4P_TIME(pr.t5);
      ++pr.kt;
#endif
    };
    int t = 0;
    for (; t + 2 < T; ++t) ktile(t, G4B<true>{}, G4B<true>{});
    if (t + 1 < T) ktile(t++, G4B<false>{}, G4B<true>{});
    ktile(t, G4B<false>{}, G4B<false>{});
    }

#ifdef GEMM_STAMPS
    if (tid == 0) {
      st[6] = __builtin_amdgcn_s_memrealtime();
      st[7] = __builtin_amdgcn_s_memtime();
    }
#endif
    asm volatile("s_nop 7\n\ts_nop 7\n\ts_nop 7" ::: "memory");
#ifdef GEMM_PROBE
    {
      unsigned long long e;
      G4P_TIME(e);
      g4_sync_lds();
      G4P_FENCE(e); G4P_FENCE(pr.loop0);
      pr.loop += e - pr.loop0;
    }
#endif
#pragma unroll
    for (int i = 0; i < 8; ++i)
      asm volatile("" : "+a"(acc[i][0]), "+a"(acc[i][1]), "+a"(acc[i][2]), "+a"(acc[i][3]),
                   "+a"(acc[i][4]), "+a"(acc[i][5]), "+a"(acc[i][6]), "+a"(acc[i][7]));

    const int crow = m0 + wr * 128 + fr;
    const int cq = 4 * (lane >> 4);
    if constexpr (F8) {
#pragma unroll
      for (int i = 0; i < 8; ++i) {
        const float sa = MXIN ? 1.f : a_scale[min(crow + i * 16, M - 1)];
#pragma unroll
        for (int j = 0; j < 8; ++j) {
          const f32x4 sb = *reinterpret_cast<const f32x4*>(b_scale + n0 + wc * 128 + j * 16 + cq);
          acc[i][j] = acc[i][j] * sb * sa;
        }
      }
    }
    if constexpr (EPI == kG4SwiGLUMx) {
      float* red = reinterpret_cast<float*>(smem + kRedOff);
#pragma unroll
      for (int i = 0; i < 8; ++i) {
        float a = 0.f;
#pragma unroll
        for (int p = 0; p < 4; ++p)
#pragma unroll
          for (int e = 0; e < 4; ++e) {
            const float g = (float)(bf16)acc[i][2 * p][e];
            const float u = (float)(bf16)acc[i][2 * p + 1][e];
            const float h = (float)(bf16)(g4_silu(g) * u);
            acc[i][2 * p][e] = h;
            a = fmaxf(a, fabsf(h));
          }
        a = fmaxf(a, __shfl_xor(a, 16, 64));
        a = fmaxf(a, __shfl_xor(a, 32, 64));
        if (lane < 16) red[wc * 256 + wr * 128 + i * 16 + fr] = a;
      }
      g4_sync_lds();
      g4_barrier();
      uint8_t* out = reinterpret_cast<uint8_t*>(C);
      const int I = N >> 1, tn = n0 >> 8;
#pragma unroll
      for (int i = 0; i < 8; ++i) {
        const int r = wr * 128 + i * 16 + fr, row = m0 + r;
        const int k = mx_exponent(fmaxf(red[r], red[256 + r]));
        const float inv = mx_inv_scale(k);
        if (row < M) {
#pragma unroll
          for (int p = 0; p < 4; ++p) {
            const f32x4 v = acc[i][2 * p] * inv;
            *reinterpret_cast<unsigned*>(out + (size_t)row * I + (n0 >> 1) + wc * 64 + p * 16 + cq) =
                pack4_fp8(v[0], v[1], v[2], v[3]);
          }
        }
        if (wc == 0 && lane < 16 && row < mx.nb * 64)
          mx.out_sc[mx_off(tn, row, mx.nb)] = (uint8_t)(row < M ? k + 127 : 127);
      }
      g4_barrier();
      continue;
    }
    if constexpr (EPI == kG4SwiGLU) {
      bf16* out = reinterpret_cast<bf16*>(C);
      const int I = N >> 1;
#pragma unroll
      for (int i = 0; i < 8; ++i) {
        const int row = crow + i * 16;
        if (row >= M) continue;
#pragma unroll
        for (int p = 0; p < 4; ++p) {
          bf16x4 o;
#pragma unroll
          for (int e = 0; e < 4; ++e) {
            const float g = (float)(bf16)acc[i][2 * p][e];
            const float u = (float)(bf16)acc[i][2 * p + 1][e];
            o[e] = (bf16)(g4_silu(g) * u);
          }
          *reinterpret_cast<bf16x4*>(out + (size_t)row * I + (n0 >> 1) + wc * 64 + p * 16 + cq) = o;
        }
      }
    } else if constexpr (EPI == kG4F32) {
      float* out = reinterpret_cast<float*>(C) + (size_t)split * M * N;
#pragma unroll
      for (int i = 0; i < 8; ++i) {
        const int row = crow + i * 16;
        if (row >= M) continue;
#pragma unroll
        for (int j = 0; j < 8; ++j)
          *reinterpret_cast<f32x4*>(out + (size_t)row * N + n0 + wc * 128 + j * 16 + cq) = acc[i][j];
      }
    } else {
      bf16* out = reinterpret_cast<bf16*>(C) + (EPI == kG4Bf16Part ? (size_t)split * M * N : 0);
#pragma unroll
      for (int i = 0; i < 8; ++i) {
        const int row = crow + i * 16;
        if (row >= M) continue;
#pragma unroll
        for (int j = 0; j < 8; ++j) {
          bf16x4 o;
#pragma unroll
          for (int e = 0; e < 4; ++e) o[e] = (bf16)acc[i][j][e];
          *reinterpret_cast<bf16x4*>(out + (size_t)row * N + n0 + wc * 128 + j * 16 + cq) = o;
        }
      }
    }
    g4_barrier();
  }
#ifdef GEMM_PROBE
  if (lane == 0) {
    unsigned long long* q = g_probe + ((size_t)blockIdx.x * 4 + w) * 8;
    q[0] = pr.b1; q[1] = pr.b2; q[2] = pr.ew; q[3] = pr.loop; q[4] = pr.kt;
  }
#endif
#ifdef GEMM_STAMPS
  if (tid == 0) {
    st[2] = __builtin_amdgcn_s_memrealtime();
    st[3] = __builtin_amdgcn_s_memtime();
  }
#endif
}

int g4_cus() {
  int dev = 0, n = 0;
  if (hipGetDevice(&dev) != hipSuccess) return 256;
  if (hipDeviceGetAttribute(&n, hipDeviceAttributeMultiprocessorCount, dev) != hipSuccess || n <= 0)
    return 256;
  return n;
}

}

int gemm4_grid(int items, int cus) {
  if (items <= cus) return items;
  const int rounds = (items + cus - 1) / cus;
  return (items + rounds - 1) / rounds;
}

template <int VAR, int PREC>
static int launch_gemm4_v(void* C, const void* a, const void* b, int M, int N, int K, int tiles_m,
                          int tiles_n, int kps, int splits, int epilogue, int grid,
                          hipStream_t stream, const float* sa, const float* sb, G4Mx mx) {
  switch (epilogue) {
    case kG4Bf16:
      gemm4_kernel<kG4Bf16, VAR, PREC><<<grid, kG4Threads, 0, stream>>>(a, b, C, M, N, K, tiles_m, tiles_n, kps, splits, sa, sb, mx);
      break;
    case kG4F32:
      gemm4_kernel<kG4F32, VAR, PREC><<<grid, kG4Threads, 0, stream>>>(a, b, C, M, N, K, tiles_m, tiles_n, kps, splits, sa, sb, mx);
      break;
    case kG4SwiGLU:
      if constexpr (PREC == 2) return -4;
      else gemm4_kernel<kG4SwiGLU, VAR, PREC><<<grid, kG4Threads, 0, stream>>>(a, b, C, M, N, K, tiles_m, tiles_n, kps, splits, sa, sb, mx);
      break;
    case kG4SwiGLUMx:
      if constexpr (PREC != 1) return -4;
      else gemm4_kernel<kG4SwiGLUMx, VAR, PREC><<<grid, kG4Threads, 0, stream>>>(a, b, C, M, N, K, tiles_m, tiles_n, kps, splits, sa, sb, mx);
      break;
    case kG4Bf16Part:
      gemm4_kernel<kG4Bf16Part, VAR, PREC><<<grid, kG4Threads, 0, stream>>>(a, b, C, M, N, K, tiles_m, tiles_n, kps, splits, sa, sb, mx);
      break;
    default:
// ... 66 lines not shown
```

distributed_llm_inference/csrc/kernels/gemm_tile.hip:

```cpp
#include "kernels.h"

namespace dli {

namespace {

constexpr int kTM = 256, kTN = 256, kTK = 64, kThreads = 512;
constexpr int kHalf = 128 * 128;
constexpr int kBuf = 4 * kHalf;
constexpr int kLds = 2 * kBuf;

enum Epilogue { kStoreBf16 = 0, kStoreF32 = 1, kSwiGLU = 2, kSwiGLUMx = 3, kStoreBf16Part = 4 };

constexpr int kSkMaxWgs = 1020, kSkErrWord = 1023, kSkHeaderFloats = 1024;

typedef __attribute__((address_space(3))) void lds_void_t;
typedef __attribute__((address_space(1))) void gbl_void_t;

__device__ __forceinline__ void dma16(const void* g, char* lds_wave_base) {
  __builtin_amdgcn_global_load_lds((gbl_void_t*)g, (lds_void_t*)lds_wave_base, 16, 0, 0);
}

__device__ __forceinline__ void dma16_nt(const void* g, char* lds_wave_base) {
  __builtin_amdgcn_global_load_lds((gbl_void_t*)g, (lds_void_t*)lds_wave_base, 16, 0, 2);
}

__device__ __forceinline__ void barrier() {
  asm volatile("" ::: "memory");
  __builtin_amdgcn_s_barrier();
  asm volatile("" ::: "memory");
}

__device__ __forceinline__ f32x4 mfma(const bf16x8& a, const bf16x8& b, const f32x4& c) {
  return __builtin_amdgcn_mfma_f32_16x16x32_bf16(a, b, c, 0, 0, 0);
}

__device__ __forceinline__ float silu(float x) { return x / (1.f + __expf(-x)); }

typedef int i32x8 __attribute__((ext_vector_type(8)));

__device__ __forceinline__ f32x4 mfma_fp8(const bf16x8& a0, const bf16x8& a1, const bf16x8& b0,
                                          const bf16x8& b1, const f32x4& c) {
  typedef int i32x4_t __attribute__((ext_vector_type(4)));
  const i32x4_t al = __builtin_bit_cast(i32x4_t, a0), ah = __builtin_bit_cast(i32x4_t, a1);
  const i32x4_t bl = __builtin_bit_cast(i32x4_t, b0), bh = __builtin_bit_cast(i32x4_t, b1);
  const i32x8 a = {al[0], al[1], al[2], al[3], ah[0], ah[1], ah[2], ah[3]};
  const i32x8 b = {bl[0], bl[1], bl[2], bl[3], bh[0], bh[1], bh[2], bh[3]};
  return __builtin_amdgcn_mfma_scale_f32_16x16x128_f8f6f4(a, b, c, 0, 0, 0, 127, 0, 127);
}

__device__ __forceinline__ f32x4 mfma_i8(const bf16x8& a, const bf16x8& b, const f32x4& c) {
  typedef int i32x4_t __attribute__((ext_vector_type(4)));
  return __builtin_bit_cast(f32x4, __builtin_amdgcn_mfma_i32_16x16x64_i8(
      __builtin_bit_cast(i32x4_t, a), __builtin_bit_cast(i32x4_t, b),
      __builtin_bit_cast(i32x4_t, c), 0, 0, 0));
}

enum Prec { kBf16 = 0, kFp8 = 1, kInt8 = 2, kFp8Mx = 3 };

template <int SEL>
__device__ __forceinline__ f32x4 mfma_fp8_mx(const bf16x8& a0, const bf16x8& a1, const bf16x8& b0,
                                             const bf16x8& b1, const f32x4& c, int sc) {
  typedef int i32x4_t __attribute__((ext_vector_type(4)));
  const i32x4_t al = __builtin_bit_cast(i32x4_t, a0), ah = __builtin_bit_cast(i32x4_t, a1);
  const i32x4_t bl = __builtin_bit_cast(i32x4_t, b0), bh = __builtin_bit_cast(i32x4_t, b1);
  const i32x8 a = {al[0], al[1], al[2], al[3], ah[0], ah[1], ah[2], ah[3]};
  const i32x8 b = {bl[0], bl[1], bl[2], bl[3], bh[0], bh[1], bh[2], bh[3]};
  return __builtin_amdgcn_mfma_scale_f32_16x16x128_f8f6f4(a, b, c, 0, 0, 0, 127, SEL, sc);
}

constexpr int kMxMaxKt = 64;
constexpr int kMxLds = kMxMaxKt * 256;

struct MxArgs {
  const uint8_t* a_sc;
  uint8_t* out_sc;
  int nb;
};

struct SkArgs {
  int n_dp;
  int sk_wgs;
  unsigned* flags;
  unsigned* err;
  float* slabs;
  int gm = 8;
};

struct OutlierArgs {
  const bf16* x;
  const bf16* w;
  int J;
  const int* cnt;
};

typedef __attribute__((address_space(1))) unsigned gu32;
typedef unsigned u32x4 __attribute__((ext_vector_type(4)));

#ifdef GEMM_STAMPS
__device__ unsigned long long* g_stamp_blk;
#endif

template <int EPI, int PREC, bool SKT, int VAR = 0>
__global__ void __launch_bounds__(kThreads, 1)
gemm_tile_kernel(const void* __restrict__ Av, const void* __restrict__ Bv, void* __restrict__ C,
                 const float* __restrict__ a_scale, const float* __restrict__ b_scale,
                 int M, int N, int K, int tiles_m, int tiles_n, int k_tiles_per_split, SkArgs sk,
                 OutlierArgs ol, MxArgs mx) {
  constexpr bool MX = PREC == kFp8Mx;
  constexpr bool FP8 = PREC == kFp8 || MX;
  constexpr bool BYTES = PREC != kBf16;
  const char* A = reinterpret_cast<const char*>(Av);
  const char* B = reinterpret_cast<const char*>(Bv);
  const size_t Kb = (size_t)K * (BYTES ? 1 : 2);
  const int kt_all = (int)(Kb / 128);
  __shared__ __attribute__((aligned(1024))) char smem[kLds + (MX ? kMxLds : 0)];

  const int tid0 = threadIdx.x;
#ifdef GEMM_STAMPS
  if (tid0 == 0) {
// ... 238 lines not shown
    int npred = 0;
    if (kSk && finish)
      for (int p = lid - 1; p >= 0; --p) {
        ++npred;
        if (sk_total * p / sk.sk_wgs <= tile_k0) break;
      }
    {
      for (int q = 1; q <= npred; ++q) {
        const int p = lid - q;
        if (__builtin_amdgcn_readfirstlane(tid >> 6) == 0) {
          unsigned spins = 0;
          while (__builtin_amdgcn_readfirstlane(__hip_atomic_load(
                     (gu32*)(sk.flags + p), __ATOMIC_RELAXED, __HIP_MEMORY_SCOPE_AGENT)) == 0u) {
            __builtin_amdgcn_s_sleep(2);
            if (++spins == (1u << 20)) {
              if (tid == 0) atomicAdd(sk.err, 1u);
              break;
            }
          }
          __builtin_amdgcn_fence(__ATOMIC_ACQUIRE, "agent");
          asm volatile("s_waitcnt vmcnt(0)" ::: "memory");
        }
        __syncthreads();
        const auto rs = __builtin_amdgcn_make_buffer_rsrc(sk.slabs + (size_t)p * (kTM * kTN), 0,
                                                          kTM * kTN * 4, 0x00020000);
#pragma unroll
        for (int i = 0; i < 8; ++i) {
          f32x4 v[4];
#pragma unroll
          for (int j = 0; j < 4; ++j)
            v[j] = __builtin_bit_cast(f32x4, __builtin_amdgcn_raw_buffer_load_b128(
                                                 rs, tid * 16, (i * 4 + j) * kThreads * 16, 0));
#pragma unroll
          for (int j = 0; j < 4; ++j) acc[i][j] += v[j];
          __builtin_amdgcn_sched_barrier(0);
        }
      }
    }

    const int crow = m0 + wr * 128 + fr;
    const int cq = 4 * (lane >> 4);
    if (BYTES) {
#pragma unroll
      for (int i = 0; i < 8; ++i) {
        const float sa = MX ? 1.f : a_scale[min(crow + i * 16, M - 1)];
#pragma unroll
        for (int j = 0; j < 4; ++j) {
          const f32x4 sb = *reinterpret_cast<const f32x4*>(b_scale + n0 + wc * 64 + j * 16 + cq);
          f32x4 v = acc[i][j];
          if (PREC == kInt8) {
            typedef int i32x4_t __attribute__((ext_vector_type(4)));
            const i32x4_t iv = __builtin_bit_cast(i32x4_t, v);
            v = f32x4{(float)iv[0], (float)iv[1], (float)iv[2], (float)iv[3]};
          }
          acc[i][j] = v * sb * sa;
        }
      }
    }
    if constexpr (PREC == kInt8) {
      if (ol.J > 0 && split == 0) {
        const int jl = ol.cnt ? min(ol.J, (*ol.cnt + 31) & ~31) : ol.J;
        for (int kk = 0; kk < jl; kk += 32) {
          bf16x8 wf[4];
#pragma unroll
          for (int j = 0; j < 4; ++j)
            wf[j] = *reinterpret_cast<const bf16x8*>(
                ol.w + (size_t)(n0 + wc * 64 + j * 16 + fr) * ol.J + kk + 8 * (lane >> 4));
#pragma unroll
          for (int i = 0; i < 8; ++i) {
            const int m = min(crow + i * 16, M - 1);
            const bf16x8 xf = *reinterpret_cast<const bf16x8*>(ol.x + (size_t)m * ol.J + kk +
                                                               8 * (lane >> 4));
#pragma unroll
            for (int j = 0; j < 4; ++j) acc[i][j] = mfma(wf[j], xf, acc[i][j]);
          }
        }
      }
    }
    if constexpr (EPI == kSwiGLUMx) {
      float* red = reinterpret_cast<float*>(smem);
#pragma unroll
      for (int i = 0; i < 8; ++i) {
        float a = 0.f;
#pragma unroll
        for (int p = 0; p < 2; ++p)
#pragma unroll
          for (int e = 0; e < 4; ++e) {
            const float g = (float)(bf16)acc[i][2 * p][e];
            const float u = (float)(bf16)acc[i][2 * p + 1][e];
            const float h = (float)(bf16)(silu(g) * u);
            acc[i][2 * p][e] = h;
            a = fmaxf(a, fabsf(h));
          }
        a = fmaxf(a, __shfl_xor(a, 16, 64));
        a = fmaxf(a, __shfl_xor(a, 32, 64));
        if (lane < 16) red[(wr * 4 + wc) * 128 + i * 16 + fr] = a;
      }
      __syncthreads();
      uint8_t* out = reinterpret_cast<uint8_t*>(C);
      const int I = N >> 1;
      const int tn = n0 / kTN;
#pragma unroll
      for (int i = 0; i < 8; ++i) {
        const int row = crow + i * 16;
        float a = 0.f;
#pragma unroll
        for (int w = 0; w < 4; ++w) a = fmaxf(a, red[(wr * 4 + w) * 128 + i * 16 + fr]);
        const int k = mx_exponent(a);
        const float inv = mx_inv_scale(k);
        if (row < M) {
#pragma unroll
          for (int p = 0; p < 2; ++p) {
            const f32x4 v = acc[i][2 * p] * inv;
            *reinterpret_cast<unsigned*>(out + (size_t)row * I + (n0 >> 1) + wc * 32 + p * 16 + cq) =
                pack4_fp8(v[0], v[1], v[2], v[3]);
          }
        }
        if (wc == 0 && lane < 16 && row < mx.nb * 64)
          mx.out_sc[mx_off(tn, row, mx.nb)] = (uint8_t)(row < M ? k + 127 : 127);
      }
    } else if (EPI == kSwiGLU) {
      bf16* out = reinterpret_cast<bf16*>(C);
      const int I = N >> 1;
#pragma unroll
      for (int i = 0; i < 8; ++i) {
        const int row = crow + i * 16;
        if (row >= M) continue;
#pragma unroll
        for (int p = 0; p < 2; ++p) {
          bf16x4 o;
#pragma unroll
          for (int e = 0; e < 4; ++e) {
            const float g = (float)(bf16)acc[i][2 * p][e];
            const float u = (float)(bf16)acc[i][2 * p + 1][e];
            o[e] = (bf16)(silu(g) * u);
          }
          *reinterpret_cast<bf16x4*>(out + (size_t)row * I + (n0 >> 1) + wc * 32 + p * 16 + cq) = o;
        }
      }
    } else if (EPI == kStoreBf16Part) {
      bf16* out = reinterpret_cast<bf16*>(C) + (size_t)split * M * N;
#pragma unroll
      for (int i = 0; i < 8; ++i) {
        const int row = crow + i * 16;
        if (row >= M) continue;
#pragma unroll
        for (int j = 0; j < 4; ++j) {
          bf16x4 o;
#pragma unroll
          for (int e = 0; e < 4; ++e) o[e] = (bf16)acc[i][j][e];
          *reinterpret_cast<bf16x4*>(out + (size_t)row * N + n0 + wc * 64 + j * 16 + cq) = o;
        }
      }
    } else if (EPI == kStoreF32) {
      float* out = reinterpret_cast<float*>(C) + (size_t)split * M * N;
#pragma unroll
      for (int i = 0; i < 8; ++i) {
        const int row = crow + i * 16;
        if (row >= M) continue;
#pragma unroll
        for (int j = 0; j < 4; ++j)
          *reinterpret_cast<f32x4*>(out + (size_t)row * N + n0 + wc * 64 + j * 16 + cq) = acc[i][j];
      }
    } else {
      bf16* out = reinterpret_cast<bf16*>(C);
#pragma unroll
      for (int i = 0; i < 8; ++i) {
        const int row = crow + i * 16;
        if (row >= M) continue;
#pragma unroll
        for (int j = 0; j < 4; ++j) {
          bf16x4 o;
#pragma unroll
          for (int e = 0; e < 4; ++e) o[e] = (bf16)acc[i][j][e];
          *reinterpret_cast<bf16x4*>(out + (size_t)row * N + n0 + wc * 64 + j * 16 + cq) = o;
        }
      }
    }
  }
#ifdef GEMM_STAMPS
  if (tid0 == 0) {
    unsigned long long* st = g_stamp_blk + (size_t)blockIdx.x * 8;
    st[2] = __builtin_amdgcn_s_memrealtime();
    st[3] = __builtin_amdgcn_s_memtime();
  }
#endif
}

__global__ void __launch_bounds__(256) tile_splitk_reduce_kernel(bf16* __restrict__ C,
                                                                 const float* __restrict__ part,
                                                                 int splits, size_t MN) {
  for (size_t i = (blockIdx.x * (size_t)blockDim.x + threadIdx.x) * 8; i < MN;
       i += (size_t)gridDim.x * blockDim.x * 8) {
    f32x4 s0 = *reinterpret_cast<const f32x4*>(part + i);
    f32x4 s1 = *reinterpret_cast<const f32x4*>(part + i + 4);
    for (int k = 1; k < splits; ++k) {
      s0 += *reinterpret_cast<const f32x4*>(part + k * MN + i);
      s1 += *reinterpret_cast<const f32x4*>(part + k * MN + i + 4);
    }
    bf16x8 o;
#pragma unroll
    for (int j = 0; j < 4; ++j) {
      o[j] = (bf16)s0[j];
      o[j + 4] = (bf16)s1[j];
    }
    *reinterpret_cast<bf16x8*>(C + i) = o;
  }
}

int device_cus() {
  static int cus[64] = {0};
  int dev = 0;
  if (hipGetDevice(&dev) != hipSuccess || dev < 0 || dev >= 64) return 0;
  if (cus[dev] == 0) {
    int n = 0;
    if (hipDeviceGetAttribute(&n, hipDeviceAttributeMultiprocessorCount, dev) != hipSuccess) return 0;
    cus[dev] = n;
  }
  return cus[dev];
// ... 140 lines not shown
```

distributed_llm_inference/csrc/kernels/kernels.h:

```cpp
#pragma once
#include "common.h"

namespace dli {

struct AttnParams {
  const bf16* q;
  const bf16* q_sink;
  const void* k_cache;
  const void* v_cache;
  int kv_fp8;
  float k_scale, v_scale;
  bf16* out;
  const int* block_tables;
  int bt_stride;
  const int* seq_lens;
  const int* q_start;
  const int* tile_map;
  int n_tiles;
  int prefill_qb = 1;
  int prefill_m32 = 1;
  float scale_log2;
  int nh, nkv, bs;
  int n_sink, sink_pad, ring, window;
  float* part_o;
  float* part_ml;
  int num_splits;
  uint8_t* out_q = nullptr;
  uint8_t* out_mx = nullptr;
  const float* mask = nullptr;
  int mask_heads = 0, mask_q = 0, mask_k = 0;
};

struct RopeCacheParams {
  const bf16* qkv;
  long qkv_stride;
  const int* positions;
  const long* slot_mapping;
  const float* cos_sin;
  int max_pos;
  bf16* q_out;
  bf16* q_sink_out;
  int window;
  void* k_cache;
  void* v_cache;
  int kv_fp8;
  float k_inv_scale, v_inv_scale;
  int nh, nkv, D, bs;
  const void* qkv_parts;
  int parts_bf16;
  int splits;
  long split_stride;
};

struct SampleParams {
  const void* logits;
  int logits_is_f32;
  long row_stride;
  int V;
  const float* temperature;
  const int* top_k;
  const float* top_p;
  const unsigned long long* seeds;
  const long* step;
  const long* ctr;
  int* out_tokens;
  float* out_logprobs;
};

int launch_rms_norm(bf16* out, const bf16* x, const bf16* residual_in, bf16* residual_out,
                    const bf16* w, float eps, int rows, int hidden, hipStream_t stream,
                    const void* x_parts = nullptr, int splits = 0, bool parts_bf16 = false);
int launch_layer_norm(bf16* out, const bf16* x, const bf16* residual_in, bf16* residual_out,
                      const bf16* w, const bf16* b, float eps, int rows, int hidden,
                      hipStream_t stream);
int launch_silu_mul(bf16* out, const bf16* x, int rows, int inter, bool interleaved,
                    hipStream_t stream);
int launch_gelu_bias(bf16* out, const bf16* x, const bf16* bias, int rows, int cols,
                     hipStream_t stream);
int launch_add(bf16* out, const bf16* a, const bf16* b, size_t n, hipStream_t stream);
int launch_digest(const void* data, long nwords, int64_t* part, int nblocks, hipStream_t stream);
int launch_rope_cache(const RopeCacheParams& p, int num_tokens, hipStream_t stream);
int launch_attn_decode(const AttnParams& p, int B, int D, hipStream_t stream);
int launch_attn_prefill(const AttnParams& p, int B, int max_q, int D, hipStream_t stream);
bool attn_prefill32_eligible(const AttnParams& p, int D);
int launch_attn_prefill32(const AttnParams& p, int B, int max_q, hipStream_t stream);
int launch_sample(const SampleParams& p, int B, hipStream_t stream);
int launch_gemm_tile(void* C, const void* A, const void* B, const float* a_scale,
                     const float* b_scale, float* workspace, int M, int N, int K, int splits,
                     int epilogue, int precision, hipStream_t stream,
                     const bf16* x_out = nullptr, const bf16* w_out = nullptr, int J = 0,
                     const uint8_t* a_mx = nullptr, uint8_t* out_mx = nullptr,
                     const int* ol_cnt = nullptr);
int launch_splitk_reduce(bf16* C, const float* parts, int splits, size_t MN, hipStream_t stream);
long long gemm_tile_sk_workspace_floats();
struct GemvNorm {
  const bf16* res_in;
  bf16* res_out;
  const bf16* w;
  float eps;
};
struct GemvRope {
  const int* positions;
  const long* slot_mapping;
  const float* cos_sin;
  int max_pos;
  bf16* q_out;
  void* k_cache;
  void* v_cache;
  int kv_fp8;
  float k_inv_scale, v_inv_scale;
  int nh, nkv, D, bs;
};
int launch_skinny_gemm_fp8(bf16* y, const void* x, const float* xscale, const uint8_t* W,
                           const float* wscale, const bf16* bias, int M, int N, int K,
                           hipStream_t stream, bool swiglu = false, const GemvNorm* nm = nullptr,
                           const GemvRope* rp = nullptr);
int launch_skinny_gemm_int8(bf16* y, const bf16* x, const int8_t* W, const float* wscale,
                            const bf16* bias, int M, int N, int K, hipStream_t stream,
                            bool swiglu = false, const GemvNorm* nm = nullptr,
                            const GemvRope* rp = nullptr);
int launch_skinny_gemm(bf16* y, const bf16* x, const bf16* W, const bf16* bias, int M, int N,
                       int K, hipStream_t stream, bool swiglu = false,
                       const GemvNorm* nm = nullptr, const GemvRope* rp = nullptr);
int launch_skinny_gemm_fp4(bf16* y, const bf16* x, const uint8_t* W, const uint8_t* bscale,
                           const bf16* bias, int M, int N, int K, hipStream_t stream,
                           bool swiglu = false, const GemvNorm* nm = nullptr,
                           const GemvRope* rp = nullptr);
int launch_dequant_mxfp4(bf16* out, const uint8_t* W, const uint8_t* bscale, size_t nblocks,
                         hipStream_t stream);
int launch_small_gemm_fp4(bf16* y, const bf16* x, const uint8_t* W, const uint8_t* bscale,
                          const bf16* bias, int M, int N, int K, bool swiglu,
                          hipStream_t stream);
int launch_small_gemm_fp8(bf16* y, const bf16* x, const uint8_t* W, const float* wscale,
                          const bf16* bias, int M, int N, int K, bool swiglu,
                          hipStream_t stream);
int launch_gemm_fp4(void* C, const uint8_t* a_q, const uint8_t* a_mx, const uint8_t* W,
                    const uint8_t* bscale, float* workspace, int M, int N, int K, int splits,
                    int epilogue, hipStream_t stream);
int gemm_fp4_max_ktiles();
int launch_quant_mx(uint8_t* q, uint8_t* sc, const bf16* x, int rows, int K, hipStream_t stream);
int launch_gemm4(void* C, const void* A, const void* B, int M, int N, int K, int splits,
                 int epilogue, int grid, hipStream_t stream, int variant = -1, int precision = 0,
                 const float* a_scale = nullptr, const float* b_scale = nullptr,
                 const uint8_t* a_mx = nullptr, uint8_t* out_mx = nullptr);
int gemm4_grid(int items, int cus);
int launch_quant_rowwise(uint8_t* q, float* scale, const bf16* x, const bf16* residual_in,
                         bf16* residual_out, const bf16* norm_w, float eps, int rows, int K,
                         hipStream_t stream, const void* x_parts = nullptr, int splits = 0,
                         bool parts_bf16 = false);
int launch_quant_rowwise_int8(int8_t* q, float* scale, const bf16* x, const uint8_t* outlier,
                              int rows, int K, hipStream_t stream);
int launch_llm_int8_colmax(float* colmax, const bf16* x, int rows, int K, hipStream_t stream);
int launch_llm_int8_select(const float* colmax, int K, float threshold, int max_out, long* idx,
                           float* sel, uint8_t* flags, hipStream_t stream, int* cnt = nullptr);
int launch_llm_int8_gather_w(bf16* w_out, const int8_t* wq, const float* ws, const long* idx,
                             const float* sel, int N, int K, int max_out, hipStream_t stream,
                             const int* cnt = nullptr);
int launch_llm_int8_gather_wt(bf16* w_out, const int8_t* wqT, const float* ws, const long* idx,
                              const float* sel, int N, int max_out, hipStream_t stream,
                              const int* cnt = nullptr);
int launch_llm_int8_gather_x(bf16* x_out, const bf16* x, const long* idx, const float* sel, int M,
                             int K, int max_out, hipStream_t stream, const int* cnt = nullptr);
int launch_silu_mul_quant(uint8_t* q, float* scale, const bf16* x, int rows, int inter,
                          hipStream_t stream);

// ... 2 lines not shown
```

distributed_llm_inference/csrc/kernels/rope_cache.hip:

```cpp
#include "kernels.h"

namespace dli {


__device__ __forceinline__ void rotate4(const bf16x4& a, const bf16x4& b, const float* cs,
                                        int i, int half, bf16x4& oa, bf16x4& ob) {
#pragma unroll
  for (int j = 0; j < 4; ++j) {
    const float c = cs[i + j], s = cs[half + i + j];
    const float x = (float)a[j], y = (float)b[j];
    oa[j] = (bf16)__builtin_fmaf(x, c, -(y * s));
    ob[j] = (bf16)__builtin_fmaf(y, c, x * s);
  }
}

template <int NS>
__device__ __forceinline__ bf16x4 load_qkv4(const RopeCacheParams& p, const bf16* row, int t,
                                            int c) {
  if constexpr (NS == 0) {
    return *reinterpret_cast<const bf16x4*>(row + c);
  } else {
    bf16x4 o;
    const size_t off = (size_t)t * p.qkv_stride + c;
    if (p.parts_bf16)
// ... 17 lines not shown
                                p.split_stride);
}

#ifndef ROPE_HPW
#define ROPE_HPW 8
#endif
constexpr int kHeadsPerWG = ROPE_HPW;

template <bool FP8, int NS>
__global__ void __launch_bounds__(128) rope_cache_kernel(RopeCacheParams p) {
  const int t = blockIdx.x;
  const int h_lo = blockIdx.y * kHeadsPerWG;
  const int D = p.D, half = D >> 1;
  const int gpr = half >> 2;
  const bf16* row = p.qkv + (size_t)t * p.qkv_stride;
  const int pos = p.positions ? p.positions[t] : 0;
  const float* cs = nullptr;
  const float* cs_sink = nullptr;
  if (p.cos_sin) {
    int pc = pos < 0 ? 0 : (pos >= p.max_pos ? p.max_pos - 1 : pos);
    cs = p.cos_sin + (size_t)pc * D;
    if (p.q_sink_out) {
      int ps = pos < p.window - 1 ? pos : p.window - 1;
      ps = ps < 0 ? 0 : (ps >= p.max_pos ? p.max_pos - 1 : ps);
      cs_sink = p.cos_sin + (size_t)ps * D;
    }
  }
  const long slot = p.slot_mapping ? p.slot_mapping[t] : -1;
  const long blk = slot >= 0 ? slot / p.bs : 0;
  const int off = slot >= 0 ? (int)(slot % p.bs) : 0;

  const int n_qk = p.nh + p.nkv;
  const int h_hi = min(h_lo + kHeadsPerWG, n_qk + p.nkv);

  const int rot_lo = h_lo * gpr, rot_hi = min(h_hi, n_qk) * gpr;
  for (int it = rot_lo + threadIdx.x; it < rot_hi; it += blockDim.x) {
    const int head = it / gpr;
    const int i = (it % gpr) * 4;
    const bf16x4 a = load_qkv4<NS>(p, row, t, head * D + i);
    const bf16x4 b = load_qkv4<NS>(p, row, t, head * D + half + i);
    bf16x4 oa = a, ob = b;
    if (cs) rotate4(a, b, cs, i, half, oa, ob);
    if (head < p.nh) {
      bf16* dst = p.q_out + ((size_t)t * p.nh + head) * D;
      *reinterpret_cast<bf16x4*>(dst + i) = oa;
      *reinterpret_cast<bf16x4*>(dst + half + i) = ob;
      if (p.q_sink_out) {
        bf16x4 sa = a, sb = b;
        if (cs_sink) rotate4(a, b, cs_sink, i, half, sa, sb);
        bf16* ds = p.q_sink_out + ((size_t)t * p.nh + head) * D;
        *reinterpret_cast<bf16x4*>(ds + i) = sa;
        *reinterpret_cast<bf16x4*>(ds + half + i) = sb;
      }
    } else if (slot >= 0) {
      const int kh = head - p.nh;
      const size_t base = (((size_t)blk * p.nkv + kh) * p.bs + off) * D;
      if (FP8) {
        uint8_t* dst = static_cast<uint8_t*>(p.k_cache) + base;
        const float s = p.k_inv_scale;
        *reinterpret_cast<unsigned*>(dst + i) =
            pack4_fp8((float)oa[0] * s, (float)oa[1] * s, (float)oa[2] * s, (float)oa[3] * s);
        *reinterpret_cast<unsigned*>(dst + half + i) =
            pack4_fp8((float)ob[0] * s, (float)ob[1] * s, (float)ob[2] * s, (float)ob[3] * s);
      } else {
        bf16* dst = static_cast<bf16*>(p.k_cache) + base;
        *reinterpret_cast<bf16x4*>(dst + i) = oa;
        *reinterpret_cast<bf16x4*>(dst + half + i) = ob;
      }
    }
  }
  if (slot >= 0 && h_hi > n_qk) {
    const int v_lo = max(h_lo - n_qk, 0) * D, v_hi = (h_hi - n_qk) * D;
    const int vcol = n_qk * D;
    const size_t grp = ((size_t)blk * p.nkv) * (p.bs >> 3) + (off >> 3);
    for (int it = v_lo + threadIdx.x; it < v_hi; it += blockDim.x) {
      const int kh = it / D, d = it % D;
      const size_t e = ((grp + (size_t)kh * (p.bs >> 3)) * D + d) * 8 + (off & 7);
      const bf16 v = load_qkv1<NS>(p, row, t, vcol + it);
      if (FP8)
        static_cast<uint8_t*>(p.v_cache)[e] = f32_to_fp8((float)v * p.v_inv_scale);
      else
        static_cast<bf16*>(p.v_cache)[e] = v;
    }
  }
}

__device__ __forceinline__ void rotate8(const bf16x8& a, const bf16x8& b, const float* cs,
                                        int i, int half, bf16x8& oa, bf16x8& ob) {
#pragma unroll
  for (int j = 0; j < 8; ++j) {
    const float c = cs[i + j], s = cs[half + i + j];
    const float x = (float)a[j], y = (float)b[j];
    oa[j] = (bf16)__builtin_fmaf(x, c, -(y * s));
    ob[j] = (bf16)__builtin_fmaf(y, c, x * s);
  }
}

template <int NS>
__device__ __forceinline__ bf16x8 load_qkv8(const RopeCacheParams& p, const bf16* row, int t,
                                            int c) {
  if constexpr (NS == 0) {
    return *reinterpret_cast<const bf16x8*>(row + c);
  } else {
    bf16x8 o;
    const size_t off = (size_t)t * p.qkv_stride + c;
    if (p.parts_bf16)
      sum_parts8<NS>(static_cast<const bf16*>(p.qkv_parts) + off, p.split_stride, o);
    else
      sum_parts8<NS>(static_cast<const float*>(p.qkv_parts) + off, p.split_stride, o);
    return o;
  }
}

#ifndef ROPE_THREADS
#define ROPE_THREADS 64
#endif
template <bool FP8, int NS>
__global__ void __launch_bounds__(ROPE_THREADS) rope_cache_kernel_v8(RopeCacheParams p) {
  const int t = blockIdx.x;
  const int h_lo = blockIdx.y * kHeadsPerWG;
  const int D = p.D, half = D >> 1;
  const int gpr = half >> 3;
  const bf16* row = p.qkv + (size_t)t * p.qkv_stride;
  const int pos = p.positions ? p.positions[t] : 0;
  const float* cs = nullptr;
  const float* cs_sink = nullptr;
  if (p.cos_sin) {
    int pc = pos < 0 ? 0 : (pos >= p.max_pos ? p.max_pos - 1 : pos);
    cs = p.cos_sin + (size_t)pc * D;
    if (p.q_sink_out) {
      int ps = pos < p.window - 1 ? pos : p.window - 1;
      ps = ps < 0 ? 0 : (ps >= p.max_pos ? p.max_pos - 1 : ps);
      cs_sink = p.cos_sin + (size_t)ps * D;
    }
  }
  const long slot = p.slot_mapping ? p.slot_mapping[t] : -1;
  const long blk = slot >= 0 ? slot / p.bs : 0;
  const int off = slot >= 0 ? (int)(slot % p.bs) : 0;
  const int n_qk = p.nh + p.nkv;
  const int h_hi = min(h_lo + kHeadsPerWG, n_qk + p.nkv);

  const int rot_lo = h_lo * gpr, rot_hi = min(h_hi, n_qk) * gpr;
  for (int it = rot_lo + threadIdx.x; it < rot_hi; it += blockDim.x) {
    const int head = it / gpr;
    const int i = (it % gpr) * 8;
    const bf16x8 a = load_qkv8<NS>(p, row, t, head * D + i);
    const bf16x8 b = load_qkv8<NS>(p, row, t, head * D + half + i);
    bf16x8 oa = a, ob = b;
    if (cs) rotate8(a, b, cs, i, half, oa, ob);
    if (head < p.nh) {
      bf16* dst = p.q_out + ((size_t)t * p.nh + head) * D;
      *reinterpret_cast<bf16x8*>(dst + i) = oa;
      *reinterpret_cast<bf16x8*>(dst + half + i) = ob;
      if (p.q_sink_out) {
        bf16x8 sa = a, sb = b;
        if (cs_sink) rotate8(a, b, cs_sink, i, half, sa, sb);
        bf16* ds = p.q_sink_out + ((size_t)t * p.nh + head) * D;
        *reinterpret_cast<bf16x8*>(ds + i) = sa;
        *reinterpret_cast<bf16x8*>(ds + half + i) = sb;
      }
    } else if (slot >= 0) {
      const int kh = head - p.nh;
      const size_t base = (((size_t)blk * p.nkv + kh) * p.bs + off) * D;
      if (FP8) {
        uint8_t* dst = static_cast<uint8_t*>(p.k_cache) + base;
        const float s = p.k_inv_scale;
        uint2 va, vb;
        va.x = pack4_fp8((float)oa[0] * s, (float)oa[1] * s, (float)oa[2] * s, (float)oa[3] * s);
        va.y = pack4_fp8((float)oa[4] * s, (float)oa[5] * s, (float)oa[6] * s, (float)oa[7] * s);
        vb.x = pack4_fp8((float)ob[0] * s, (float)ob[1] * s, (float)ob[2] * s, (float)ob[3] * s);
        vb.y = pack4_fp8((float)ob[4] * s, (float)ob[5] * s, (float)ob[6] * s, (float)ob[7] * s);
        *reinterpret_cast<uint2*>(dst + i) = va;
        *reinterpret_cast<uint2*>(dst + half + i) = vb;
      } else {
        bf16* dst = static_cast<bf16*>(p.k_cache) + base;
        *reinterpret_cast<bf16x8*>(dst + i) = oa;
        *reinterpret_cast<bf16x8*>(dst + half + i) = ob;
// ... 55 lines not shown
```

distributed_llm_inference/models/llama/modules.py:

```python
from __future__ import annotations

from typing import Optional, Tuple

import torch
import torch.nn as nn

from ... import ops
from ...config import ModelSpec
from ..common import AttnMetadata, Linear


def rotate_half(x: torch.Tensor) -> torch.Tensor:
    x1, x2 = x.chunk(2, dim=-1)
    return torch.cat((-x2, x1), dim=-1)


def apply_rotary_pos_emb(q: torch.Tensor, k: torch.Tensor, cos: torch.Tensor, sin: torch.Tensor,
                         unsqueeze_dim: int = 1) -> Tuple[torch.Tensor, torch.Tensor]:
    c = cos.unsqueeze(unsqueeze_dim).float()
    s = sin.unsqueeze(unsqueeze_dim).float()
    qf, kf = q.float(), k.float()
    return ((qf * c + rotate_half(qf) * s).to(q.dtype), (kf * c + rotate_half(kf) * s).to(k.dtype))


class RMSNorm(nn.Module):
    def __init__(self, hidden: int, eps: float, device=None, dtype=torch.bfloat16):
        super().__init__()
        self.weight = nn.Parameter(torch.ones(hidden, dtype=dtype, device=device), requires_grad=False)
        self.eps = eps

    def forward(self, x: torch.Tensor, residual: Optional[torch.Tensor] = None,
                residual_out: Optional[torch.Tensor] = None):
        return ops.rms_norm(x, self.weight, self.eps, residual=residual, residual_out=residual_out)


class LlamaAttention(nn.Module):
    def __init__(self, spec: ModelSpec, layer_idx: int, device=None, dtype=torch.bfloat16):
        super().__init__()
        self.layer_idx = layer_idx
        self.num_heads = spec.num_heads
        self.num_kv_heads = spec.num_kv_heads
        self.head_dim = spec.head_dim
        self.scale = spec.head_dim ** -0.5
        self.qkv_proj = Linear(spec.hidden_size, spec.qkv_size, bias=spec.attention_bias,
                               dtype=dtype, device=device)
        self.o_proj = Linear(spec.q_size, spec.hidden_size, bias=spec.has_o_proj_bias, dtype=dtype,
                             device=device)
        self.qkv_proj.role, self.o_proj.role = "qkv", "o"

    def forward(self, normed: Optional[torch.Tensor], meta: AttnMetadata, k_cache: torch.Tensor,
                v_cache: torch.Tensor, cos_sin: torch.Tensor, x_q=None, defer_reduce: bool = False,
                norm: Optional[ops.RowNorm] = None):
        q = None
        if norm is not None:
            q = self.qkv_proj.gemv_qkv_rope(normed, meta, k_cache, v_cache, cos_sin,
                                            self.num_heads, self.num_kv_heads, self.head_dim,
                                            norm=norm)
            q_sink = None
            if q is None:
                qkv = self.qkv_proj.gemv(normed, norm=norm)
                if qkv is None:
                    raise RuntimeError("fused-norm QKV: the GEMV does not take this product")
        else:
            qkv = self.qkv_proj(normed, x_q, defer_reduce=True)
        if q is None:
            q, q_sink = ops.rope_cache(qkv, meta.positions, meta.slot_mapping, cos_sin,
                                       self.num_heads, self.num_kv_heads, self.head_dim, k_cache,
                                       v_cache, window=meta.window, want_sink=meta.want_sink,
                                       k_scale=meta.k_scale, v_scale=meta.v_scale)
        T = q.shape[0]
        if meta.custom_mask is not None:
            o = ops.attn_prefill(q, None, k_cache, v_cache, meta.block_tables, meta.seq_lens,
                                 meta.q_start, meta.max_q, self.scale, k_scale=meta.k_scale,
                                 v_scale=meta.v_scale, mask=meta.custom_mask)
        elif meta.is_decode:
            op = self.o_proj
            mx = (op.is_fp8 and op.bias is None and ops.policy().fp8_mx
                  and ops.attn_decode_mx_ok(self.head_dim, meta.num_splits)
                  and not op.fp8_small_rows(T))
            if mx and q.is_cuda:
                sp = ops.tile_gemm_splits_fp8(T, op.out_features, op.in_features)
                mx = bool(sp) and ops.mx_tileable(op.in_features, sp)
            if mx:
                o = ops.attn_decode(q, q_sink, k_cache, v_cache, meta.block_tables, meta.seq_lens,
                                    self.scale, meta.n_sink, meta.sink_pad, meta.ring, meta.window,
                                    num_splits=meta.num_splits, workspace=meta.workspace,
                                    k_scale=meta.k_scale, v_scale=meta.v_scale, mx_out=True)
                return op(None, x_q=o, defer_reduce=defer_reduce)
            o = ops.attn_decode(q, q_sink, k_cache, v_cache, meta.block_tables, meta.seq_lens,
                                self.scale, meta.n_sink, meta.sink_pad, meta.ring, meta.window,
                                num_splits=meta.num_splits, workspace=meta.workspace,
                                k_scale=meta.k_scale, v_scale=meta.v_scale)
        else:
            o = ops.attn_prefill(q, q_sink, k_cache, v_cache, meta.block_tables, meta.seq_lens,
                                 meta.q_start, meta.max_q, self.scale, meta.n_sink, meta.sink_pad,
                                 meta.ring, meta.window, k_scale=meta.k_scale,
                                 v_scale=meta.v_scale, tile_map=meta.tile_map)
        o = o.view(T, self.num_heads * self.head_dim)
        return self.o_proj(o, defer_reduce=defer_reduce)


class LlamaMLP(nn.Module):
    def __init__(self, spec: ModelSpec, device=None, dtype=torch.bfloat16):
        super().__init__()
        if spec.hidden_act != "silu":
            raise ValueError(f"unsupported Llama activation {spec.hidden_act!r}")
        self.intermediate_size = spec.intermediate_size
        self.gate_up_proj = Linear(spec.hidden_size, 2 * spec.intermediate_size, bias=spec.mlp_bias,
                                   dtype=dtype, device=device)
        self.down_proj = Linear(spec.intermediate_size, spec.hidden_size, bias=spec.mlp_bias,
                                dtype=dtype, device=device)
        self.gate_up_proj.role, self.down_proj.role = "gate_up", "down"
        self.fused_swiglu = False

    def set_fused_swiglu(self, on: bool) -> None:
        w = self.gate_up_proj
        if on == self.fused_swiglu:
            return
        if w.bias is not None or w.out_features % 256:
            return
        perm = ops.swiglu_interleave if on else ops.swiglu_deinterleave
        with torch.no_grad():
            if w.is_int8:
                w.weight_int8.copy_(perm(w.weight_int8))
                w.weight_scale.copy_(perm(w.weight_scale.reshape(-1, 1)).reshape(w.weight_scale.shape))
                if w.weight_int8_t is not None:
                    w.weight_int8_t.copy_(perm(w.weight_int8_t.t()).t())
            elif w.is_fp4:
                w.weight_fp4.copy_(perm(w.weight_fp4))
                w.weight_block_scale.copy_(perm(w.weight_block_scale))
            elif w.is_fp8:
                w.weight_fp8.copy_(perm(w.weight_fp8.view(torch.uint8)).view(w.weight_fp8.dtype))
                w.weight_scale.copy_(perm(w.weight_scale.reshape(-1, 1)).reshape(w.weight_scale.shape))
            else:
                w.weight.data.copy_(perm(w.weight.data))
        self.fused_swiglu = on

    def forward(self, normed: Optional[torch.Tensor], x_q=None, defer_reduce: bool = False,
                norm: Optional[ops.RowNorm] = None):
        gp = self.gate_up_proj
        if norm is not None:
            h = gp.gemv(normed, swiglu=True, norm=norm)
            if h is None:
                raise RuntimeError("fused-norm gate|up: the GEMV does not take this product")
            return self.down_proj(h, defer_reduce=defer_reduce)
        if self.fused_swiglu and ops.policy().gemv:
            h = gp.gemv_swiglu(normed, x_q)
            if h is not None:
                return self.down_proj(h, defer_reduce=defer_reduce)
        if self.fused_swiglu and gp.is_int8:
            h = ops.llm_int8_linear(normed, gp.weight_int8, gp.weight_scale, gp.int8_threshold,
                                    wq_t=gp.weight_int8_t, swiglu=True)
            return self.down_proj(h, defer_reduce=defer_reduce)
        if (self.fused_swiglu and gp.bias is None and x_q is None
                and gp.fp8_small_ok(normed)):
            h = ops.small_gemm_fp8(normed, gp.weight_fp8, gp.weight_scale, swiglu=True)
            return self.down_proj(h, defer_reduce=defer_reduce)
        if self.fused_swiglu and gp.is_fp8:
            xq, xs = x_q if x_q is not None else ops.quant_rowwise(normed)
            if xq.is_cuda and ops.tile_gemm_splits_fp8(xq.shape[0], gp.out_features,
                                                        gp.in_features):
                dp = self.down_proj
                dsp = ops.tile_gemm_splits_fp8(xq.shape[0], dp.out_features, dp.in_features)
                g4 = ops.policy().fp8_on_gemm4("gate_up")
                if (ops.policy().fp8_mx and dsp and dp.bias is None
                        and ops.mx_tileable(dp.in_features, dsp)):
# ... 168 lines not shown
```

distributed_llm_inference/ops/__init__.py:

```python
from __future__ import annotations

import contextlib
import math
import os
from typing import Optional, Tuple

import torch

from ..config import KernelPolicy
from . import reference as ref

_C = None
_POLICY: Optional[KernelPolicy] = None


def policy() -> KernelPolicy:
    global _POLICY
    if _POLICY is None:
        _POLICY = KernelPolicy().with_overrides(os.environ.get("DLI_KERNELS", ""))
    return _POLICY


def set_policy(p: KernelPolicy) -> KernelPolicy:
    global _POLICY
# ... 139 lines not shown
               q_sink_out: Optional[torch.Tensor] = None, k_scale: float = 1.0,
               v_scale: float = 1.0):
    if isinstance(qkv, SplitKPartials):
        T = qkv.shape[0]
        if q_out is None:
            q_out = torch.empty(T, nh, head_dim, dtype=torch.bfloat16, device=qkv.device)
        if want_sink and q_sink_out is None:
            q_sink_out = torch.empty_like(q_out)
        native().rope_cache(qkv.parts, positions, slot_mapping, cos_sin, q_out,
                            q_sink_out if want_sink else None, int(window), k_cache, v_cache,
                            int(nh), int(nkv), float(k_scale), float(v_scale))
        return q_out, (q_sink_out if want_sink else None)
    if not _gpu(qkv):
        q, qs = ref.rope_cache(qkv, positions, slot_mapping, cos_sin, nh, nkv, head_dim, k_cache,
                               v_cache, window, want_sink, k_scale, v_scale)
        if q_out is not None:
            q_out.copy_(q)
            q = q_out
        if qs is not None and q_sink_out is not None:
            q_sink_out.copy_(qs)
            qs = q_sink_out
        return q, qs
    T = qkv.shape[0]
    if q_out is None:
        q_out = torch.empty(T, nh, head_dim, dtype=qkv.dtype, device=qkv.device)
    if want_sink and q_sink_out is None:
        q_sink_out = torch.empty_like(q_out)
    native().rope_cache(qkv, positions, slot_mapping, cos_sin, q_out,
                        q_sink_out if want_sink else None, int(window), k_cache, v_cache,
                        int(nh), int(nkv), float(k_scale), float(v_scale))
    return q_out, (q_sink_out if want_sink else None)


def decode_splits(batch: int, nkv: int, group: int, max_len: int, cu: int = 256,
                  kv_fp8: bool = False) -> int:
    waves = batch * nkv * ((group + 15) // 16)
    if waves >= 8 * cu:
        return 1
    target = 4 * cu
    want = (target + waves - 1) // waves
    max_useful = max(1, (max_len + 31) // 32)
    s = int(max(1, min(want, max_useful, 512)))
    if kv_fp8 and 2 <= s <= 16:
        s = min(2 * s, max_useful)
    if s >= 4:
        return s // 4 * 4
    return 2 if s == 3 else s


def attn_decode_mx_ok(head_dim: int, num_splits: int) -> bool:
    return head_dim == 128 and num_splits == 1


def attn_decode(q, q_sink, k_cache, v_cache, block_tables, seq_lens, scale, n_sink=0, sink_pad=0,
                ring=0, window=0, num_splits=1, workspace=None, out=None, k_scale=1.0, v_scale=1.0,
                mx_out: bool = False):
    if mx_out and not attn_decode_mx_ok(q.shape[-1], num_splits):
        raise ValueError("attn_decode(mx_out=True) needs head_dim 128 and one split")
    if not _gpu(q):
        y = ref.attn_decode(q, q_sink, k_cache, v_cache, block_tables, seq_lens, scale, n_sink,
                            sink_pad, ring, window, k_scale, v_scale)
        if mx_out:
            return mx_quantize(y.to(torch.bfloat16).reshape(q.shape[0], -1))
        return out.copy_(y) if out is not None else y
    if mx_out:
        T, nh, D = q.shape
        nb = (T + 63) // 64
        q8 = torch.empty(T, nh * D, dtype=torch.float8_e4m3fn, device=q.device)
        sc = torch.empty(nh * nb * 64, dtype=torch.uint8, device=q.device)
        dummy = q.new_empty((0, nh, D))
        native().attn_decode(dummy, q, q_sink, k_cache, v_cache, block_tables, seq_lens,
                             float(scale), int(n_sink), int(sink_pad), int(ring), int(window), 1,
                             None, None, float(k_scale), float(v_scale), q8, sc)
        return MxFp8(q8, sc)
    out = torch.empty_like(q) if out is None else out
    part_o = part_ml = None
    if num_splits > 1:
        if workspace is None:
            workspace = decode_workspace(q.shape[0], q.shape[1], q.shape[2], num_splits, q.device)
        part_o, part_ml = workspace[0], workspace[1]
    native().attn_decode(out, q, q_sink, k_cache, v_cache, block_tables, seq_lens, float(scale),
                         int(n_sink), int(sink_pad), int(ring), int(window), int(num_splits),
                         part_o, part_ml, float(k_scale), float(v_scale))
    return out


def decode_workspace(rows: int, nh: int, head_dim: int, splits: int, device):
    return (torch.empty(splits * rows * nh * head_dim, dtype=torch.float32, device=device),
            torch.empty(splits * rows * nh * 2, dtype=torch.float32, device=device))


PREFILL_QB = 1
PREFILL_QB_LONG = 1024


def prefill_qb_for(max_q: int) -> int:
    return 2 if max_q >= PREFILL_QB_LONG else PREFILL_QB


def prefill_tile_tokens(nh: int, nkv: int, qb: int = PREFILL_QB) -> int:
    G = nh // nkv
    hpw = 4 if G % 4 == 0 else (2 if G % 2 == 0 else 1)
    return 16 * (4 // hpw) * qb


def prefill_tiles(q_lens, nh: int, nkv: int, out=None, qb: Optional[int] = None) -> torch.Tensor:
    import numpy as np
    if qb is None:
        qb = prefill_qb_for(max(q_lens) if len(q_lens) else 0)
    tt = prefill_tile_tokens(nh, nkv, qb)
    ql = np.asarray(q_lens, dtype=np.int64)
    nt = (ql + tt - 1) // tt
    b = np.repeat(np.arange(len(ql), dtype=np.int32), nt)
    starts = np.repeat(np.cumsum(nt) - nt, nt)
    tile = (np.arange(int(nt.sum())) - starts).astype(np.int32)
    m = np.stack([b, tile], axis=1)
    if out is not None:
        out.numpy()[: len(m)] = m
        return out[: len(m)]
    return torch.from_numpy(np.ascontiguousarray(m))


def attn_prefill(q, q_sink, k_cache, v_cache, block_tables, seq_lens, q_start, max_q, scale,
                 n_sink=0, sink_pad=0, ring=0, window=0, out=None, k_scale=1.0, v_scale=1.0,
                 tile_map=None, mask=None, qb: Optional[int] = None):
    if not _gpu(q):
        if mask is not None:
            y = ref.attn_custom_mask(q, k_cache, v_cache, block_tables, seq_lens, q_start, scale,
                                     mask, k_scale, v_scale)
        else:
            y = ref.attn_prefill(q, q_sink, k_cache, v_cache, block_tables, seq_lens, q_start,
                                 scale, n_sink, sink_pad, ring, window, k_scale, v_scale)
        return out.copy_(y) if out is not None else y
    out = torch.empty_like(q) if out is None else out
    if qb is None:
        qb = prefill_qb_for(int(max_q))
    if mask is not None:
        if ring:
            raise ValueError("custom 4-D masks need a full (non-windowed) cache")
        mask = mask.to(device=q.device, dtype=torch.float32).contiguous()
        tile_map = None
    native().attn_prefill(out, q, q_sink, k_cache, v_cache, block_tables, seq_lens, q_start,
                          int(max_q), float(scale), int(n_sink), int(sink_pad), int(ring),
                          int(window), float(k_scale), float(v_scale), tile_map, int(qb), mask,
                          bool(policy().prefill_m32))
    return out


def digest(t: torch.Tensor, nblocks: int = 256) -> torch.Tensor:
    if not _gpu(t) or (t.numel() * t.element_size()) % 4:
        return ref.digest_parts(t)
    t = t.contiguous()
    part = torch.empty(nblocks, 2, dtype=torch.int64, device=t.device)
    native().digest(part, t)
    return part


digest_fold = ref.digest_fold


def sample(logits: torch.Tensor, temperature: Optional[torch.Tensor] = None,
           top_k: Optional[torch.Tensor] = None, top_p: Optional[torch.Tensor] = None,
           seeds: Optional[torch.Tensor] = None, step: Optional[torch.Tensor] = None,
           out: Optional[torch.Tensor] = None, logprobs: Optional[torch.Tensor] = None,
           generator: Optional[torch.Generator] = None,
           counters: Optional[torch.Tensor] = None) -> torch.Tensor:
# ... 752 lines not shown
```

Before: 6962 tokens/s.

## Fold RoPE and KV-cache write into one-step decode attention; faster bf16 SiLU

Adds an opt-in decode attention variant that reads the raw QKV projection, or split-K partials, directly. It applies RoPE in a wave prologue and writes K/V into the paged cache, so the separate rope_cache kernel and its q round-trip through memory go away. The variant is gated by a new fused_rope_attn policy flag, which defaults to off, and only runs for one-step, bf16-cache, D=128 shapes. Separately, the SwiGLU activation and a GEMM epilogue switch to a vectorised silu_mul_bf16 helper, and a probe kernel is added to compare it against the plain silu. The fused path adds more work per wave, and the faster SiLU may change numerics slightly.

Result: no change. 6958 tokens/s (-0.1%).

```diff
diff --git a/distributed_llm_inference/config.py b/distributed_llm_inference/config.py
--- a/distributed_llm_inference/config.py
+++ b/distributed_llm_inference/config.py
@@ -353,6 +353,7 @@
     fp4_mfma: bool = False
     fp4_small_m: int = 0
     fp8_small_m: int = 0
+    fused_rope_attn: bool = False
 
     _FP8_SHAPES = ("qkv", "o", "gate_up", "down")
 
diff --git a/distributed_llm_inference/csrc/bindings.hip b/distributed_llm_inference/csrc/bindings.hip
--- a/distributed_llm_inference/csrc/bindings.hip
+++ b/distributed_llm_inference/csrc/bindings.hip
@@ -128,6 +128,19 @@
   check_rc(dli::launch_silu_mul(bp(out), bp(x), (int)rows, (int)(two_i / 2), interleaved,
                                 cur_stream()),
            "silu_mul");
+}
+
+void silu_probe(Tensor fast, Tensor plain, Tensor x) {
+  CHECK_IN(fast); CHECK_IN(plain); CHECK_IN(x); CHECK_BF16(x);
+  TORCH_CHECK(fast.scalar_type() == at::kInt && plain.scalar_type() == at::kInt,
+              "silu_probe: outputs must be int32");
+  TORCH_CHECK(fast.numel() == x.numel() && plain.numel() == x.numel() && x.numel() % 8 == 0,
+              "silu_probe: shape mismatch");
+  const c10::hip::HIPGuardMasqueradingAsCUDA g(x.device());
+  check_rc(dli::launch_silu_probe(reinterpret_cast<unsigned*>(fast.data_ptr()),
+                                  reinterpret_cast<unsigned*>(plain.data_ptr()), bp(x),
+                                  (int)x.numel(), cur_stream()),
+           "silu_probe");
 }
 
 void gelu_bias(Tensor out, Tensor x, optional<Tensor> bias) {
@@ -323,6 +336,77 @@
   const c10::hip::HIPGuardMasqueradingAsCUDA g(q.device());
   check_rc(dli::launch_attn_decode(p, (int)B, (int)D, cur_stream()), "attn_decode");
 }
+
+void attn_decode_rope(Tensor out, Tensor qkv, optional<Tensor> positions,
+                      optional<Tensor> slot_mapping, optional<Tensor> cos_sin, Tensor k_cache,
+                      Tensor v_cache, Tensor block_tables, Tensor seq_lens, double scale,
+                      int64_t nh, bool force) {
+  CHECK_DEV(qkv);
+  const bool parts_bf16 = qkv.scalar_type() == at::kBFloat16 && qkv.dim() == 3;
+  const bool parts = qkv.scalar_type() == at::kFloat || parts_bf16;
+  if (parts) {
+    TORCH_CHECK(qkv.dim() == 3 && qkv.is_contiguous(), "qkv partials must be contiguous [S, T, N]");
+  } else {
+    CHECK_BF16(qkv);
+    TORCH_CHECK(qkv.dim() == 2 && qkv.stride(1) == 1, "qkv must be [T, *] with unit inner stride");
+  }
+  const int64_t T = parts ? qkv.size(1) : qkv.size(0);
+  CHECK_IN(out); CHECK_BF16(out);
+  TORCH_CHECK(out.dim() == 3 && out.size(0) == T && out.size(1) == nh && out.size(2) == 128,
+              "attn_decode_rope: out must be [T, nh, 128]");
+  const int64_t D = 128, nkv = k_cache.size(1);
+  TORCH_CHECK(nkv > 0 && nh % nkv == 0 && nh / nkv <= 16, "attn_decode_rope: GQA group of 1..16");
+  TORCH_CHECK(qkv.size(qkv.dim() - 1) >= (nh + 2 * nkv) * D, "qkv too narrow for nh/nkv/D");
+  TORCH_CHECK(!check_cache(k_cache, v_cache, nkv, D), "attn_decode_rope: bf16 KV cache only");
+  CHECK_IN(block_tables); CHECK_I32(block_tables); CHECK_IN(seq_lens); CHECK_I32(seq_lens);
+  TORCH_CHECK(block_tables.dim() == 2 && block_tables.size(0) == T && seq_lens.numel() == T,
+              "decode: one token per sequence (block_tables [T, max_blocks], seq_lens [T])");
+  dli::AttnParams p{};
+  if (parts) {
+    p.qkv_parts = qkv.data_ptr();
+    p.parts_bf16 = parts_bf16 ? 1 : 0;
+    p.qkv_splits = (int)qkv.size(0);
+    p.qkv_stride = qkv.size(2);
+    p.split_stride = (long)(T * qkv.size(2));
+  } else {
+    p.qkv = bp(qkv);
+    p.qkv_stride = qkv.stride(0);
+  }
+  if (positions.has_value()) {
+    CHECK_IN(*positions); CHECK_I32(*positions);
+    TORCH_CHECK(positions->numel() == T, "positions must have T entries");
+    p.positions = positions->data_ptr<int>();
+  }
+  if (slot_mapping.has_value()) {
+    CHECK_IN(*slot_mapping); CHECK_I64(*slot_mapping);
+    TORCH_CHECK(slot_mapping->numel() == T, "slot_mapping must have T entries");
+    p.slot_mapping = reinterpret_cast<const long*>(slot_mapping->data_ptr<int64_t>());
+  }
+  if (cos_sin.has_value()) {
+    CHECK_IN(*cos_sin); CHECK_F32(*cos_sin);
+    TORCH_CHECK(cos_sin->dim() == 2 && cos_sin->size(1) == D, "cos_sin must be [max_pos, D]");
+    TORCH_CHECK(positions.has_value(), "rope needs positions");
+    p.cos_sin = cos_sin->data_ptr<float>();
+    p.max_pos = (int)cos_sin->size(0);
+  }
+  p.k_cache = k_cache.data_ptr();
+  p.v_cache = v_cache.data_ptr();
+  p.k_scale = p.v_scale = 1.f;
+  p.out = bp(out);
+  p.block_tables = block_tables.data_ptr<int>();
+  p.bt_stride = (int)block_tables.size(1);
+  p.seq_lens = seq_lens.data_ptr<int>();
+  p.scale_log2 = (float)(scale * 1.4426950408889634);
+  p.nh = (int)nh;
+  p.nkv = (int)nkv;
+  p.bs = (int)k_cache.size(2);
+  p.num_splits = 1;
+  TORCH_CHECK(p.bs % 32 == 0, "cache block size must be a multiple of 32");
+  const c10::hip::HIPGuardMasqueradingAsCUDA g(qkv.device());
+  check_rc(dli::launch_attn_decode_rope(p, (int)T, force, cur_stream()), "attn_decode_rope");
+}
+
+bool attn_one_step(int64_t items) { return dli::attn_decode_one_step((long)items); }
 
 void attn_prefill(Tensor out, Tensor q, optional<Tensor> q_sink, Tensor k_cache, Tensor v_cache,
                   Tensor block_tables, Tensor seq_lens, Tensor q_start, int64_t max_q,
@@ -1095,6 +1179,7 @@
         py::arg("residual_out") = py::none());
   m.def("silu_mul", &silu_mul, "SwiGLU: out = silu(x[:, :I]) * x[:, I:] (or tile-interleaved)",
         py::arg("out"), py::arg("x"), py::arg("interleaved") = false);
+  m.def("silu_probe", &silu_probe, "test hook: silu_bf16 and silu on bf16 values, raw fp32 words");
   m.def("gelu_bias", &gelu_bias, "gelu_tanh(x + bias)");
   m.def("add", &add, "out = a + b");
   m.def("rope_cache", &rope_cache, "fused RoPE + paged KV cache write");
@@ -1104,6 +1189,13 @@
         py::arg("sink_pad"), py::arg("ring"), py::arg("window"), py::arg("num_splits"),
         py::arg("part_o"), py::arg("part_ml"), py::arg("k_scale"), py::arg("v_scale"),
         py::arg("out_q") = py::none(), py::arg("out_mx") = py::none());
+  m.def("attn_decode_rope", &attn_decode_rope,
+        "single-split bf16-KV decode attention with RoPE and the KV write folded in",
+        py::arg("out"), py::arg("qkv"), py::arg("positions"), py::arg("slot_mapping"),
+        py::arg("cos_sin"), py::arg("k_cache"), py::arg("v_cache"), py::arg("block_tables"),
+        py::arg("seq_lens"), py::arg("scale"), py::arg("nh"), py::arg("force") = false);
+  m.def("attn_one_step", &attn_one_step,
+        "whether single-split full-cache decode of this many waves runs the one-step kernel");
   m.def("attn_prefill", &attn_prefill, "paged causal prefill attention (varlen)", py::arg("out"),
         py::arg("q"), py::arg("q_sink"), py::arg("k_cache"), py::arg("v_cache"),
         py::arg("block_tables"), py::arg("seq_lens"), py::arg("q_start"), py::arg("max_q"),
diff --git a/distributed_llm_inference/csrc/kernels/activation.hip b/distributed_llm_inference/csrc/kernels/activation.hip
--- a/distributed_llm_inference/csrc/kernels/activation.hip
+++ b/distributed_llm_inference/csrc/kernels/activation.hip
@@ -22,10 +22,34 @@
       g = reinterpret_cast<const bf16x8*>(row)[c];
       u = reinterpret_cast<const bf16x8*>(row + inter)[c];
     }
+    float s[8], t[8];
+#pragma unroll
+    for (int j = 0; j < 8; ++j) {
+      s[j] = (float)g[j];
+      t[j] = (float)u[j];
+    }
+    silu_mul_bf16(s, t);
     bf16x8 o;
 #pragma unroll
-    for (int j = 0; j < 8; ++j) o[j] = (bf16)(silu((float)g[j]) * (float)u[j]);
+    for (int j = 0; j < 8; ++j) o[j] = (bf16)s[j];
     reinterpret_cast<bf16x8*>(out + r * inter)[c] = o;
+  }
+}
+
+__global__ void __launch_bounds__(256) silu_probe_kernel(unsigned* __restrict__ fast,
+                                                         unsigned* __restrict__ plain,
+                                                         const bf16* __restrict__ x, int nvec) {
+  const int i = blockIdx.x * blockDim.x + threadIdx.x;
+  if (i >= nvec) return;
+  const bf16x8 v = reinterpret_cast<const bf16x8*>(x)[i];
+  float s[8];
+#pragma unroll
+  for (int j = 0; j < 8; ++j) s[j] = (float)v[j];
+  silu_bf16(s);
+#pragma unroll
+  for (int j = 0; j < 8; ++j) {
+    fast[(size_t)i * 8 + j] = __float_as_uint(s[j]);
+    plain[(size_t)i * 8 + j] = __float_as_uint(silu((float)v[j]));
   }
 }
 
@@ -83,6 +107,13 @@
   return 0;
 }
 
+int launch_silu_probe(unsigned* fast, unsigned* plain, const bf16* x, int n, hipStream_t stream) {
+  if (n % 8 != 0) return -1;
+  if (n == 0) return 0;
+  silu_probe_kernel<<<(n / 8 + 255) / 256, 256, 0, stream>>>(fast, plain, x, n / 8);
+  return 0;
+}
+
 int launch_gelu_bias(bf16* out, const bf16* x, const bf16* bias, int rows, int cols,
                      hipStream_t stream) {
   if (cols % 8 != 0) return -1;
diff --git a/distributed_llm_inference/csrc/kernels/attention.hip b/distributed_llm_inference/csrc/kernels/attention.hip
--- a/distributed_llm_inference/csrc/kernels/attention.hip
+++ b/distributed_llm_inference/csrc/kernels/attention.hip
@@ -5,9 +5,88 @@
 
 namespace dli {
 
-template <int D, bool WIN, bool FP8, bool GRP, bool ONE = false>
+template <int NS>
+__device__ __forceinline__ bf16x8 qkv_ld8(const AttnParams& p, int t, int c) {
+  const size_t off = (size_t)t * p.qkv_stride + c;
+  if constexpr (NS == 0) {
+    return *reinterpret_cast<const bf16x8*>(p.qkv + off);
+  } else {
+    bf16x8 o;
+    if (p.parts_bf16)
+      sum_parts8<NS>(static_cast<const bf16*>(p.qkv_parts) + off, p.split_stride, o);
+    else
+      sum_parts8<NS>(static_cast<const float*>(p.qkv_parts) + off, p.split_stride, o);
+    return o;
+  }
+}
+
+template <int NS>
+__device__ __forceinline__ void rope_head(const AttnParams& p, int t, int role, int kvh, int col,
+                                          int h4, const float* cs, long slot, bf16x8 (&r)[4]) {
+  constexpr int D = 128;
+  if (role < 0) return;
+  const int G = p.nh / p.nkv;
+  const int head = role == 0 ? kvh * G + col : (role == 1 ? p.nh + kvh : p.nh + p.nkv + kvh);
+#pragma unroll
+  for (int c = 0; c < 2; ++c) {
+    const int i = 32 * c + 8 * h4;
+    const bf16x8 a = qkv_ld8<NS>(p, t, head * D + i);
+    const bf16x8 b = qkv_ld8<NS>(p, t, head * D + 64 + i);
+    bf16x8 oa = a, ob = b;
+    if (cs != nullptr && role != 2) rotate8(a, b, cs, i, 64, oa, ob);
+    r[c] = oa;
+    r[c + 2] = ob;
+  }
+  if (role == 0 || slot < 0) return;
+  const long blk = slot / p.bs;
+  const int off = (int)(slot % p.bs);
+  if (role == 1) {
+    bf16* dst = const_cast<bf16*>(static_cast<const bf16*>(p.k_cache)) +
+                (((size_t)blk * p.nkv + kvh) * p.bs + off) * D;
+#pragma unroll
+    for (int c = 0; c < 4; ++c) *reinterpret_cast<bf16x8*>(dst + 32 * c + 8 * h4) = r[c];
+  } else {
+    bf16* dst = const_cast<bf16*>(static_cast<const bf16*>(p.v_cache)) +
+                (((size_t)blk * p.nkv + kvh) * (p.bs >> 3) + (off >> 3)) * D * 8 + (off & 7);
+#pragma unroll
+    for (int c = 0; c < 4; ++c)
+#pragma unroll
+      for (int j = 0; j < 8; ++j) dst[(32 * c + 8 * h4 + j) * 8] = r[c][j];
+  }
+}
+
+template <int NS>
+__device__ __forceinline__ void rope_prologue(const AttnParams& p, int b, int kvh, bf16x8 (&qf)[4]) {
+  constexpr int D = 128;
+  const int lane = threadIdx.x & 63, col = lane & 15, h4 = lane >> 4;
+  const int G = p.nh / p.nkv;
+  const int pos = p.positions ? p.positions[b] : 0;
+  const float* cs = nullptr;
+  if (p.cos_sin) {
+    const int pc = pos < 0 ? 0 : (pos >= p.max_pos ? p.max_pos - 1 : pos);
+    cs = p.cos_sin + (size_t)pc * D;
+  }
+  const long slot = p.slot_mapping ? p.slot_mapping[b] : -1;
+  const bool spare = G + 2 <= 16;
+  const int role = col < G ? 0 : ((spare && col < G + 2) ? 1 + (col - G) : -1);
+#pragma unroll
+  for (int c = 0; c < 4; ++c) qf[c] = zero8();
+  rope_head<NS>(p, b, role, kvh, col, h4, cs, slot, qf);
+  if (role != 0) {
+#pragma unroll
+    for (int c = 0; c < 4; ++c) qf[c] = zero8();
+  }
+  if (!spare) {
+    bf16x8 r[4];
+    rope_head<NS>(p, b, col < 2 ? 1 + col : -1, kvh, col, h4, cs, slot, r);
+  }
+}
+
+template <int D, bool WIN, bool FP8, bool GRP, bool ONE = false, int ROPE = -1>
 __global__ void __launch_bounds__(256, (ONE ? 4 : 1))
 attn_decode_kernel(AttnParams p, int items, int gs) {
+  static_assert(ROPE < 0 || (D == 128 && ONE && !WIN && !FP8 && !GRP),
+                "fused RoPE: one-step, full bf16 cache, D = 128");
   constexpr int LROW = D + 4;
   __shared__ __attribute__((aligned(16))) float lds[GRP ? 4 * 16 * (LROW + 2) : 1];
   const int wave = threadIdx.x >> 6;
@@ -16,7 +95,14 @@
   if (!GRP && !live) return;
   const int item = __builtin_amdgcn_readfirstlane(live ? item_raw : items - 1);
   WaveState<D> st;
-  const DecodeItem di = attn_decode_item<D, WIN, FP8, false, ONE>(p, item, live, st);
+  DecodeItem di;
+  if constexpr (ROPE >= 0) {
+    di = attn_decode_item<D, WIN, FP8, false, ONE>(p, item, live, st, [&](bf16x8 (&qf)[4]) {
+      rope_prologue<ROPE>(p, item / p.nkv, item % p.nkv, qf);
+    });
+  } else {
+    di = attn_decode_item<D, WIN, FP8, false, ONE>(p, item, live, st);
+  }
   const int splits = p.num_splits, split = di.split, G = di.G, hgroups = di.hgroups;
   const int g0 = di.g0, kvh = di.kvh, b = di.b;
   const int lane = threadIdx.x & 63, col = lane & 15, h4 = lane >> 4;
@@ -469,6 +555,12 @@
   return cus;
 }
 
+bool attn_decode_one_step(long items) {
+  const long s1 = 16L * attn_cus(), s2 = 8L * attn_cus();
+  const long r1 = (items + s1 - 1) / s1, r2 = (items + s2 - 1) / s2;
+  return items >= s1 && (double)items / (r1 * s1) >= (double)items / (r2 * s2);
+}
+
 template <int D, bool WIN, bool FP8>
 static void decode_grid(const AttnParams& p, int items, int gs, hipStream_t stream) {
   const int grid = (items + 3) / 4;
@@ -478,9 +570,7 @@
   }
   if constexpr (!WIN) {
 #ifndef ATTN_DECODE_TWO_STEP
-    const long s1 = 16L * attn_cus(), s2 = 8L * attn_cus();
-    const long r1 = (items + s1 - 1) / s1, r2 = (items + s2 - 1) / s2;
-    if (items >= s1 && (double)items / (r1 * s1) >= (double)items / (r2 * s2)) {
+    if (attn_decode_one_step(items)) {
       attn_decode_kernel<D, WIN, FP8, false, true><<<grid, 256, 0, stream>>>(p, items, 1);
       return;
     }
@@ -508,6 +598,33 @@
     pc.num_splits = p.num_splits / gs;
     attn_combine_kernel<D><<<B * p.nh, 256, 0, stream>>>(pc, B);
   }
+  return 0;
+}
+
+int launch_attn_decode_rope(const AttnParams& p, int B, bool force, hipStream_t stream) {
+  if (B == 0) return 0;
+  if (p.bs % 32 != 0 || p.ring > 0 || p.kv_fp8 || p.num_splits != 1 || p.out_q != nullptr) return -2;
+  if (p.nkv <= 0 || p.nh % p.nkv != 0 || p.nh / p.nkv > 16) return -3;
+  const bool parts = p.qkv_parts != nullptr;
+  if ((!parts && p.qkv == nullptr) || p.qkv_stride % 8 != 0 ||
+      (parts && (p.qkv_splits < 1 || p.qkv_splits > 4 || p.split_stride % 8 != 0)))
+    return -4;
+  if (p.cos_sin != nullptr && p.positions == nullptr) return -4;
+  const long items = (long)B * p.nkv;
+  if (items > (1L << 30)) return -3;
+  if (!force && !attn_decode_one_step(items)) return -5;
+  const int grid = (int)((items + 3) / 4);
+#define ROPE_ATTN_LAUNCH(NS) \
+  attn_decode_kernel<128, false, false, false, true, NS><<<grid, 256, 0, stream>>>(p, (int)items, 1)
+  switch (parts ? p.qkv_splits : 0) {
+    case 0: ROPE_ATTN_LAUNCH(0); break;
+    case 1: ROPE_ATTN_LAUNCH(1); break;
+    case 2: ROPE_ATTN_LAUNCH(2); break;
+    case 3: ROPE_ATTN_LAUNCH(3); break;
+    case 4: ROPE_ATTN_LAUNCH(4); break;
+    default: return -4;
+  }
+#undef ROPE_ATTN_LAUNCH
   return 0;
 }
 
diff --git a/distributed_llm_inference/csrc/kernels/attn_core.h b/distributed_llm_inference/csrc/kernels/attn_core.h
--- a/distributed_llm_inference/csrc/kernels/attn_core.h
+++ b/distributed_llm_inference/csrc/kernels/attn_core.h
@@ -1,5 +1,7 @@
 #pragma once
 #include "kernels.h"
+
+#include <type_traits>
 
 namespace dli {
 
@@ -257,9 +259,19 @@
   float vsc;
 };
 
-template <int D, bool WIN, bool FP8, bool NT, bool ONE_STEP = false>
+struct NoQPre {};
+
+__device__ __forceinline__ void wave_store_load_fence() {
+  __builtin_amdgcn_fence(__ATOMIC_RELEASE, "wavefront");
+  asm volatile("s_waitcnt vmcnt(0)" ::: "memory");
+  __builtin_amdgcn_fence(__ATOMIC_ACQUIRE, "wavefront");
+}
+
+template <int D, bool WIN, bool FP8, bool NT, bool ONE_STEP = false, typename QPre = NoQPre>
 __device__ __forceinline__ DecodeItem attn_decode_item(const AttnParams& p, int item, bool live,
-                                                       WaveState<D>& st) {
+                                                       WaveState<D>& st, QPre qpre = QPre()) {
+  constexpr bool QPRE = !std::is_same<QPre, NoQPre>::value;
+  static_assert(!QPRE || (ONE_STEP && !WIN && !FP8), "q prologue: one-step full bf16 cache");
   const int splits = p.num_splits;
   const int split = item % splits;
   int rest = item / splits;
@@ -282,10 +294,12 @@
   st.init();
   if (L > 0) {
     bf16x8 qf[D / 32];
-    const bf16* qrow = p.q + ((size_t)b * p.nh + qh) * D;
-#pragma unroll
-    for (int c = 0; c < D / 32; ++c)
-      qf[c] = col_valid ? *reinterpret_cast<const bf16x8*>(qrow + q_dofs<D, FP8>(c, h4)) : zero8();
+    if constexpr (!QPRE) {
+      const bf16* qrow = p.q + ((size_t)b * p.nh + qh) * D;
+#pragma unroll
+      for (int c = 0; c < D / 32; ++c)
+        qf[c] = col_valid ? *reinterpret_cast<const bf16x8*>(qrow + q_dofs<D, FP8>(c, h4)) : zero8();
+    }
     int seg_base, seg_len;
     if (WIN) {
       seg_base = p.sink_pad;
@@ -343,11 +357,22 @@
         }
       } else {
       if constexpr (ONE_STEP) {
+        if constexpr (QPRE) {
+          qpre(qf);
+          for (int sidx = s_lo; sidx < s_hi; ++sidx) {
+            if (sidx == s_hi - 1) wave_store_load_fence();
+            KVFrag<D> f;
+            load(f, sidx);
+            attn_compute<D>(st, qf, f, sl2,
+                            step_mask<D, WIN>(seg_base + sidx * 32, h4, seg_base, seg_len, L, p));
+          }
+        } else {
         for (int sidx = s_lo; sidx < s_hi; ++sidx) {
           KVFrag<D> f;
           load(f, sidx);
           attn_compute<D>(st, qf, f, sl2,
                           step_mask<D, WIN>(seg_base + sidx * 32, h4, seg_base, seg_len, L, p));
+        }
         }
       } else {
       KVFrag<D> fa, fb;
@@ -383,6 +408,12 @@
       }
     }
   }
+  if constexpr (QPRE) {
+    if (L <= 0) {
+      bf16x8 qf[D / 32];
+      qpre(qf);
+    }
+  }
   DecodeItem di;
   di.split = split;
   di.b = b;
diff --git a/distributed_llm_inference/csrc/kernels/common.h b/distributed_llm_inference/csrc/kernels/common.h
--- a/distributed_llm_inference/csrc/kernels/common.h
+++ b/distributed_llm_inference/csrc/kernels/common.h
@@ -204,6 +204,17 @@
   }
 }
 
+__device__ __forceinline__ void rotate8(const bf16x8& a, const bf16x8& b, const float* cs,
+                                        int i, int half, bf16x8& oa, bf16x8& ob) {
+#pragma unroll
+  for (int j = 0; j < 8; ++j) {
+    const float c = cs[i + j], s = cs[half + i + j];
+    const float x = (float)a[j], y = (float)b[j];
+    oa[j] = (bf16)__builtin_fmaf(x, c, -(y * s));
+    ob[j] = (bf16)__builtin_fmaf(y, c, x * s);
+  }
+}
+
 #define SPLITS_SWITCH(splits, MACRO) \
   switch (splits) {                      \
     case 0: MACRO(0); break;             \
@@ -282,6 +293,48 @@
 
 __device__ __forceinline__ float silu(float x) { return x / (1.f + __expf(-x)); }
 
+constexpr float kSiluFastMax = 87.f;
+template <int N>
+__device__ __forceinline__ void silu_bf16(float (&x)[N]) {
+  static_assert(N % 2 == 0, "silu_bf16 works on pairs");
+  f32x2 ss = {0.f, 0.f};
+#pragma unroll
+  for (int e = 0; e < N; e += 2) {
+    const f32x2 v = {x[e], x[e + 1]};
+    ss = __builtin_elementwise_fma(v, v, ss);
+  }
+  const bool fast = ss[0] + ss[1] <= kSiluFastMax * kSiluFastMax;
+  if (__builtin_amdgcn_ballot_w64(!fast) == 0) {
+#pragma unroll
+    for (int e = 0; e < N; e += 2) {
+      const f32x2 v = {x[e], x[e + 1]};
+      const f32x2 t = v * -1.44269504088896340736f;
+      f32x2 d = {__builtin_amdgcn_exp2f(t[0]), __builtin_amdgcn_exp2f(t[1])};
+      d = d + 1.f;
+      const f32x2 r = {__builtin_amdgcn_rcpf(d[0]), __builtin_amdgcn_rcpf(d[1])};
+      const f32x2 q = v * r;
+      const f32x2 m = __builtin_elementwise_fma(q, d, -v);
+      const f32x2 y = __builtin_elementwise_fma(-m, r, q);
+      x[e] = y[0];
+      x[e + 1] = y[1];
+    }
+  } else {
+#pragma unroll
+    for (int e = 0; e < N; ++e) x[e] = silu(x[e]);
+  }
+}
+
+template <int N>
+__device__ __forceinline__ void silu_mul_bf16(float (&g)[N], const float (&u)[N]) {
+  silu_bf16(g);
+#pragma unroll
+  for (int e = 0; e < N; e += 2) {
+    const f32x2 h = f32x2{g[e], g[e + 1]} * f32x2{u[e], u[e + 1]};
+    g[e] = h[0];
+    g[e + 1] = h[1];
+  }
+}
+
 __device__ __forceinline__ float gelu_tanh(float x) {
   const float k0 = 0.7978845608028654f, k1 = 0.044715f;
   return 0.5f * x * (1.f + tanhf(k0 * (x + k1 * x * x * x)));
diff --git a/distributed_llm_inference/csrc/kernels/gemm4.hip b/distributed_llm_inference/csrc/kernels/gemm4.hip
--- a/distributed_llm_inference/csrc/kernels/gemm4.hip
+++ b/distributed_llm_inference/csrc/kernels/gemm4.hip
@@ -59,7 +59,6 @@
 };
 constexpr int kG4Default = 4, kG4DecodeDefault = 8;
 
-__device__ __forceinline__ float g4_silu(float x) { return x / (1.f + __expf(-x)); }
 
 __device__ __forceinline__ void g4_mfma(f32x4& acc, const bf16x8& w, const bf16x8& x) {
   asm volatile("v_mfma_f32_16x16x32_bf16 %0, %1, %2, %0" : "+a"(acc) : "v"(w), "v"(x) : "memory");
@@ -533,13 +532,20 @@
 #pragma unroll
       for (int i = 0; i < 8; ++i) {
         float a = 0.f;
+        float g[16], u[16];
 #pragma unroll
         for (int p = 0; p < 4; ++p)
 #pragma unroll
           for (int e = 0; e < 4; ++e) {
-            const float g = (float)(bf16)acc[i][2 * p][e];
-            const float u = (float)(bf16)acc[i][2 * p + 1][e];
-            const float h = (float)(bf16)(g4_silu(g) * u);
+            g[4 * p + e] = (float)(bf16)acc[i][2 * p][e];
+            u[4 * p + e] = (float)(bf16)acc[i][2 * p + 1][e];
+          }
+        silu_mul_bf16(g, u);
+#pragma unroll
+        for (int p = 0; p < 4; ++p)
+#pragma unroll
+          for (int e = 0; e < 4; ++e) {
+            const float h = (float)(bf16)g[4 * p + e];
             acc[i][2 * p][e] = h;
             a = fmaxf(a, fabsf(h));
           }
@@ -577,15 +583,20 @@
       for (int i = 0; i < 8; ++i) {
         const int row = crow + i * 16;
         if (row >= M) continue;
+        float g[16], u[16];
+#pragma unroll
+        for (int p = 0; p < 4; ++p)
+#pragma unroll
+          for (int e = 0; e < 4; ++e) {
+            g[4 * p + e] = (float)(bf16)acc[i][2 * p][e];
+            u[4 * p + e] = (float)(bf16)acc[i][2 * p + 1][e];
+          }
+        silu_mul_bf16(g, u);
 #pragma unroll
         for (int p = 0; p < 4; ++p) {
           bf16x4 o;
 #pragma unroll
-          for (int e = 0; e < 4; ++e) {
-            const float g = (float)(bf16)acc[i][2 * p][e];
-            const float u = (float)(bf16)acc[i][2 * p + 1][e];
-            o[e] = (bf16)(g4_silu(g) * u);
-          }
+          for (int e = 0; e < 4; ++e) o[e] = (bf16)g[4 * p + e];
           *reinterpret_cast<bf16x4*>(out + (size_t)row * I + (n0 >> 1) + wc * 64 + p * 16 + cq) = o;
         }
       }
diff --git a/distributed_llm_inference/csrc/kernels/gemm_tile.hip b/distributed_llm_inference/csrc/kernels/gemm_tile.hip
--- a/distributed_llm_inference/csrc/kernels/gemm_tile.hip
+++ b/distributed_llm_inference/csrc/kernels/gemm_tile.hip
@@ -33,8 +33,6 @@
 __device__ __forceinline__ f32x4 mfma(const bf16x8& a, const bf16x8& b, const f32x4& c) {
   return __builtin_amdgcn_mfma_f32_16x16x32_bf16(a, b, c, 0, 0, 0);
 }
-
-__device__ __forceinline__ float silu(float x) { return x / (1.f + __expf(-x)); }
 
 typedef int i32x8 __attribute__((ext_vector_type(8)));
 
@@ -439,13 +437,20 @@
 #pragma unroll
       for (int i = 0; i < 8; ++i) {
         float a = 0.f;
+        float g[8], u[8];
 #pragma unroll
         for (int p = 0; p < 2; ++p)
 #pragma unroll
           for (int e = 0; e < 4; ++e) {
-            const float g = (float)(bf16)acc[i][2 * p][e];
-            const float u = (float)(bf16)acc[i][2 * p + 1][e];
-            const float h = (float)(bf16)(silu(g) * u);
+            g[4 * p + e] = (float)(bf16)acc[i][2 * p][e];
+            u[4 * p + e] = (float)(bf16)acc[i][2 * p + 1][e];
+          }
+        silu_mul_bf16(g, u);
+#pragma unroll
+        for (int p = 0; p < 2; ++p)
+#pragma unroll
+          for (int e = 0; e < 4; ++e) {
+            const float h = (float)(bf16)g[4 * p + e];
             acc[i][2 * p][e] = h;
             a = fmaxf(a, fabsf(h));
           }
@@ -483,15 +488,20 @@
       for (int i = 0; i < 8; ++i) {
         const int row = crow + i * 16;
         if (row >= M) continue;
+        float g[8], u[8];
+#pragma unroll
+        for (int p = 0; p < 2; ++p)
+#pragma unroll
+          for (int e = 0; e < 4; ++e) {
+            g[4 * p + e] = (float)(bf16)acc[i][2 * p][e];
+            u[4 * p + e] = (float)(bf16)acc[i][2 * p + 1][e];
+          }
+        silu_mul_bf16(g, u);
 #pragma unroll
         for (int p = 0; p < 2; ++p) {
           bf16x4 o;
 #pragma unroll
-          for (int e = 0; e < 4; ++e) {
-            const float g = (float)(bf16)acc[i][2 * p][e];
-            const float u = (float)(bf16)acc[i][2 * p + 1][e];
-            o[e] = (bf16)(silu(g) * u);
-          }
+          for (int e = 0; e < 4; ++e) o[e] = (bf16)g[4 * p + e];
           *reinterpret_cast<bf16x4*>(out + (size_t)row * I + (n0 >> 1) + wc * 32 + p * 16 + cq) = o;
         }
       }
diff --git a/distributed_llm_inference/csrc/kernels/kernels.h b/distributed_llm_inference/csrc/kernels/kernels.h
--- a/distributed_llm_inference/csrc/kernels/kernels.h
+++ b/distributed_llm_inference/csrc/kernels/kernels.h
@@ -29,6 +29,14 @@
   uint8_t* out_mx = nullptr;
   const float* mask = nullptr;
   int mask_heads = 0, mask_q = 0, mask_k = 0;
+  const bf16* qkv = nullptr;
+  const void* qkv_parts = nullptr;
+  int parts_bf16 = 0, qkv_splits = 0;
+  long qkv_stride = 0, split_stride = 0;
+  const int* positions = nullptr;
+  const long* slot_mapping = nullptr;
+  const float* cos_sin = nullptr;
+  int max_pos = 0;
 };
 
 struct RopeCacheParams {
@@ -75,12 +83,15 @@
                       hipStream_t stream);
 int launch_silu_mul(bf16* out, const bf16* x, int rows, int inter, bool interleaved,
                     hipStream_t stream);
+int launch_silu_probe(unsigned* fast, unsigned* plain, const bf16* x, int n, hipStream_t stream);
 int launch_gelu_bias(bf16* out, const bf16* x, const bf16* bias, int rows, int cols,
                      hipStream_t stream);
 int launch_add(bf16* out, const bf16* a, const bf16* b, size_t n, hipStream_t stream);
 int launch_digest(const void* data, long nwords, int64_t* part, int nblocks, hipStream_t stream);
 int launch_rope_cache(const RopeCacheParams& p, int num_tokens, hipStream_t stream);
 int launch_attn_decode(const AttnParams& p, int B, int D, hipStream_t stream);
+bool attn_decode_one_step(long items);
+int launch_attn_decode_rope(const AttnParams& p, int B, bool force, hipStream_t stream);
 int launch_attn_prefill(const AttnParams& p, int B, int max_q, int D, hipStream_t stream);
 bool attn_prefill32_eligible(const AttnParams& p, int D);
 int launch_attn_prefill32(const AttnParams& p, int B, int max_q, hipStream_t stream);
diff --git a/distributed_llm_inference/csrc/kernels/rope_cache.hip b/distributed_llm_inference/csrc/kernels/rope_cache.hip
--- a/distributed_llm_inference/csrc/kernels/rope_cache.hip
+++ b/distributed_llm_inference/csrc/kernels/rope_cache.hip
@@ -123,17 +123,6 @@
       else
         static_cast<bf16*>(p.v_cache)[e] = v;
     }
-  }
-}
-
-__device__ __forceinline__ void rotate8(const bf16x8& a, const bf16x8& b, const float* cs,
-                                        int i, int half, bf16x8& oa, bf16x8& ob) {
-#pragma unroll
-  for (int j = 0; j < 8; ++j) {
-    const float c = cs[i + j], s = cs[half + i + j];
-    const float x = (float)a[j], y = (float)b[j];
-    oa[j] = (bf16)__builtin_fmaf(x, c, -(y * s));
-    ob[j] = (bf16)__builtin_fmaf(y, c, x * s);
   }
 }
 
diff --git a/distributed_llm_inference/models/llama/modules.py b/distributed_llm_inference/models/llama/modules.py
--- a/distributed_llm_inference/models/llama/modules.py
+++ b/distributed_llm_inference/models/llama/modules.py
@@ -48,6 +48,25 @@
                              device=device)
         self.qkv_proj.role, self.o_proj.role = "qkv", "o"
 
+    def _mx_out(self, T: int, meta: AttnMetadata, on_gpu: bool) -> bool:
+        op = self.o_proj
+        mx = (op.is_fp8 and op.bias is None and ops.policy().fp8_mx
+              and ops.attn_decode_mx_ok(self.head_dim, meta.num_splits)
+              and not op.fp8_small_rows(T))
+        if mx and on_gpu:
+            sp = ops.tile_gemm_splits_fp8(T, op.out_features, op.in_features)
+            mx = bool(sp) and ops.mx_tileable(op.in_features, sp)
+        return bool(mx)
+
+    def _fused_rope_attn(self, qkv, meta: AttnMetadata, k_cache: torch.Tensor) -> bool:
+        if not (ops.policy().fused_rope_attn and meta.is_decode and meta.custom_mask is None
+                and not meta.windowed and not meta.want_sink and qkv.is_cuda):
+            return False
+        if not ops.attn_decode_rope_ok(qkv, self.num_heads, self.num_kv_heads, self.head_dim,
+                                       k_cache, meta.num_splits):
+            return False
+        return not self._mx_out(qkv.shape[0], meta, True)
+
     def forward(self, normed: Optional[torch.Tensor], meta: AttnMetadata, k_cache: torch.Tensor,
                 v_cache: torch.Tensor, cos_sin: torch.Tensor, x_q=None, defer_reduce: bool = False,
                 norm: Optional[ops.RowNorm] = None):
@@ -63,6 +82,12 @@
                     raise RuntimeError("fused-norm QKV: the GEMV does not take this product")
         else:
             qkv = self.qkv_proj(normed, x_q, defer_reduce=True)
+        if q is None and self._fused_rope_attn(qkv, meta, k_cache):
+            o = ops.attn_decode_rope(qkv, meta.positions, meta.slot_mapping, cos_sin,
+                                     self.num_heads, self.num_kv_heads, self.head_dim, k_cache,
+                                     v_cache, meta.block_tables, meta.seq_lens, self.scale)
+            return self.o_proj(o.view(o.shape[0], self.num_heads * self.head_dim),
+                               defer_reduce=defer_reduce)
         if q is None:
             q, q_sink = ops.rope_cache(qkv, meta.positions, meta.slot_mapping, cos_sin,
                                        self.num_heads, self.num_kv_heads, self.head_dim, k_cache,
@@ -75,13 +100,7 @@
                                  v_scale=meta.v_scale, mask=meta.custom_mask)
         elif meta.is_decode:
             op = self.o_proj
-            mx = (op.is_fp8 and op.bias is None and ops.policy().fp8_mx
-                  and ops.attn_decode_mx_ok(self.head_dim, meta.num_splits)
-                  and not op.fp8_small_rows(T))
-            if mx and q.is_cuda:
-                sp = ops.tile_gemm_splits_fp8(T, op.out_features, op.in_features)
-                mx = bool(sp) and ops.mx_tileable(op.in_features, sp)
-            if mx:
+            if self._mx_out(T, meta, q.is_cuda):
                 o = ops.attn_decode(q, q_sink, k_cache, v_cache, meta.block_tables, meta.seq_lens,
                                     self.scale, meta.n_sink, meta.sink_pad, meta.ring, meta.window,
                                     num_splits=meta.num_splits, workspace=meta.workspace,
diff --git a/distributed_llm_inference/ops/__init__.py b/distributed_llm_inference/ops/__init__.py
--- a/distributed_llm_inference/ops/__init__.py
+++ b/distributed_llm_inference/ops/__init__.py
@@ -245,6 +245,46 @@
     native().attn_decode(out, q, q_sink, k_cache, v_cache, block_tables, seq_lens, float(scale),
                          int(n_sink), int(sink_pad), int(ring), int(window), int(num_splits),
                          part_o, part_ml, float(k_scale), float(v_scale))
+    return out
+
+
+FORCE_ATTN_DECODE_ROPE = False
+
+
+def attn_decode_rope_ok(qkv, nh: int, nkv: int, head_dim: int, k_cache: torch.Tensor,
+                        num_splits: int = 1, force: bool = False) -> bool:
+    if isinstance(qkv, SplitKPartials):
+        t = qkv.parts
+        if t.shape[0] > 4 or not t.is_contiguous():
+            return False
+        stride, rows = t.shape[2], t.shape[1]
+        aligned = stride % 8 == 0 and (rows * stride) % 8 == 0
+    else:
+        t = qkv
+        if t.dim() != 2 or t.dtype != torch.bfloat16 or t.stride(1) != 1:
+            return False
+        stride, rows = t.stride(0), t.shape[0]
+        aligned = stride % 8 == 0
+    if not t.is_cuda or not aligned or t.data_ptr() % 16:
+        return False
+    if (head_dim != 128 or num_splits != 1 or nh % nkv or nh // nkv > 16
+            or k_cache.dtype != torch.bfloat16):
+        return False
+    return bool(force or FORCE_ATTN_DECODE_ROPE) or bool(native().attn_one_step(rows * nkv))
+
+
+def attn_decode_rope(qkv, positions, slot_mapping, cos_sin, nh: int, nkv: int, head_dim: int,
+                     k_cache, v_cache, block_tables, seq_lens, scale, out=None,
+                     force: bool = False) -> torch.Tensor:
+    force = bool(force or FORCE_ATTN_DECODE_ROPE)
+    if not attn_decode_rope_ok(qkv, nh, nkv, head_dim, k_cache, 1, force):
+        raise ValueError("attn_decode_rope does not take this step (attn_decode_rope_ok)")
+    t = qkv.parts if isinstance(qkv, SplitKPartials) else qkv
+    T = qkv.shape[0]
+    if out is None:
+        out = torch.empty(T, nh, head_dim, dtype=torch.bfloat16, device=t.device)
+    native().attn_decode_rope(out, t, positions, slot_mapping, cos_sin, k_cache, v_cache,
+                              block_tables, seq_lens, float(scale), int(nh), bool(force))
     return out
 
 
```
